# One-2-3-45/One-2-3-45

Hardware: NVIDIA H100
Metric: sec/mesh end-to-end (256x256 in) (lower is better)
Workload: dtype f16

## Files before the change

include/o2345.h:

```cpp
#ifndef O2345_H_
#define O2345_H_

#include <stddef.h>
#include <stdint.h>

#ifdef __cplusplus
extern "C" {
#endif

#define O2345_OK 0
#define O2345_EINVAL (-1)
#define O2345_ECUDA (-2)
#define O2345_EUNSUPPORTED (-3)

#define O2345_ABI_VERSION 5

typedef void* o2345_stream_t;

int o2345_abi_version(void);
int o2345_last_error(char* buf, size_t n);
int o2345_device_info(int* major, int* minor, int* sms);


#define O2345_SDF_PE 39
#define O2345_SDF_HID 128
#define O2345_SDF_LAT 16
#define O2345_SDF_IN1 144
#define O2345_SDF_PACK_FLOATS (39 * 128 + 128 + 2 * (144 * 128 + 128) + 128 * 144 + 128 * 48)

int o2345_sdf_pack_weights(const float* w0, const float* b0, const float* w1, const float* b1,
                           const float* w2, const float* b2, float* pack, o2345_stream_t stream);

#define O2345_PTS_EXPLICIT 0
#define O2345_PTS_LATTICE 1
#define O2345_PTS_RAYS 2

typedef struct o2345_points {
  int mode;
  const float* pts;
  const float* lin;
  int R;
  const float* rays_o;
  const float* rays_d;
  const float* z;
  int S;
  int z_stride;
} o2345_points;

#define O2345_SDF_FP32 0
#define O2345_SDF_TC_SPLIT 1
int o2345_sdf_query(const o2345_points* src, int64_t n, const float* vol_cl, int D, const float* wpack,
                    const uint8_t* active, float inactive_sdf, int negate, int precision, float* sdf, float* feat,
                    float* latent, float* grad, o2345_stream_t stream);


int o2345_frustum_mask(const float* proj, int V, const float* origin, float voxel_size, int D, int sizeH,
                       int sizeW, int min_views, uint32_t* mask_bits, uint8_t* keep, o2345_stream_t stream);

int64_t o2345_compact_scratch_ints(int64_t n);
int o2345_compact(const uint8_t* flags, int64_t n, int32_t* rows, int32_t* index, int32_t* count,
                  int32_t* scratch, o2345_stream_t stream);

int o2345_costvol_gather(const float* feats_nhwc, int V, int h, int w, int sizeH, int sizeW, const float* proj,
                         const float* origin, float voxel_size, int D, const int32_t* rows, const int32_t* count,
                         int64_t max_rows, const uint32_t* mask_bits, float* cost, o2345_stream_t stream);

int o2345_dense_scatter(const float* feat, const int32_t* rows, const int32_t* count, int64_t max_rows, int D,
                        float* vol_cl, float* vol_cf, float* occ, o2345_stream_t stream);

int o2345_occ_nearest(const o2345_points* src, int64_t n, const float* occ, int D, uint8_t* out,
                      o2345_stream_t stream);


int o2345_sdf_voxels(const float* occ, const float* vol_cl, int D, const float* origin, float voxel_size,
                     const float* wpack, int precision, float* sdf_vol, o2345_stream_t stream);

int o2345_prune_by_sdf(const float* sdf, const float* occ, int D, const float* ladder, int n_ladder, float* scratch,
                       float* minabs, int32_t* counts, o2345_stream_t stream);
int o2345_prune_select(const float* minabs, int64_t n, float threshold, uint8_t* keep, o2345_stream_t stream);
int o2345_clear_flags(const int32_t* rows, const int32_t* idx, int64_t n, uint8_t* flags, o2345_stream_t stream);
int o2345_gather_rows(const int32_t* rows, int64_t n, int D, const float* vol_cf, int C, float* coords, float* feats,
                      o2345_stream_t stream);

int o2345_lod_children(const float* pre_coords, int64_t n, int D1, const uint8_t* frustum_keep, uint8_t* keep,
                       int32_t* parent, int32_t* err_scratch, o2345_stream_t stream);

int o2345_costvol_gather_lod(const float* feats_nhwc, int C, int V, int h, int w, int sizeH, int sizeW, const float* proj,
                             const float* origin, float voxel_size, int D, const int32_t* rows, const int32_t* count,
                             int64_t max_rows, const uint32_t* mask_bits, const int32_t* parent, const float* pre_feats,
                             float* cost, o2345_stream_t stream);


int o2345_sp_coarsen(const int32_t* fine_index, int Ef, const int32_t* fine_rows, const int32_t* fine_count,
                     int64_t max_fine, int Ec, uint8_t* coarse_flags, int32_t* cmin_scratch,
                     o2345_stream_t stream);

int o2345_sp_conv(const float* in_feats, const int32_t* in_index, int Ein, const int32_t* out_rows,
                  const int32_t* out_count, int64_t max_out, int Eout, int mode, const float* kernel, int Cin,
                  int Cout, float* out_raw, double* stats, o2345_stream_t stream);

int o2345_sp_bn_relu(const float* x, const int32_t* count, int64_t max_rows, int C, const double* stats,
                     const float* gamma, const float* beta, float eps, const float* skip, float* out,
                     o2345_stream_t stream);

int o2345_mc_classify(const float* u, int R, float iso, uint8_t* cases, uint8_t* cell_flags, uint8_t* edge_flags,
                      o2345_stream_t stream);
int o2345_mc_vertices(const float* u, int R, float iso, const int32_t* edges, const int32_t* count,
                      int64_t max_verts, double* verts, o2345_stream_t stream);
int64_t o2345_scan_scratch_ints(int64_t n);
int o2345_mc_tri_offsets(const uint8_t* cases, const int32_t* cells, const int32_t* count, int64_t max_cells,
                         const uint8_t* n_tri_table, int32_t* offsets, int32_t* total, int32_t* scratch,
                         o2345_stream_t stream);
int o2345_mc_triangles(const uint8_t* cases, int R, const int32_t* cells, const int32_t* count, int64_t max_cells,
                       const int32_t* tri_offsets, const int8_t* tri_table, const uint8_t* n_tri_table,
                       const int8_t* edge_owner, const int32_t* vert_index, int32_t* tris, o2345_stream_t stream);

typedef struct o2345_view4 {
  float* ptr;
  int64_t sn, sc, sh, sw;
  int c0;
} o2345_view4;

int o2345_conv2d(const float* in, int N, int Cin, int H, int W, const float* weight, const float* bias, int Cout,
                 int K, int stride, int pad, float* out, double* stats, o2345_stream_t stream);
int o2345_abn_apply(const float* x, int N, int C, int H, int W, const double* stats, const float* gamma,
                    const float* beta, float eps, float slope, const o2345_view4* out, o2345_stream_t stream);
int o2345_upsample_bilinear(const float* x, int N, int C, int H, int W, int factor, const float* add,
                            const o2345_view4* out, o2345_stream_t stream);


int o2345_ray_upsample(const float* rays_o, const float* rays_d, int64_t R, const float* z, const float* sdf,
                       int S, float inv_s, const float* occ, int D, const float* u, int n_new, float* new_z,
                       o2345_stream_t stream);
int o2345_ray_merge(const float* z, const float* sdf, int S, const float* new_z, const float* new_sdf, int n_new,
                    int64_t R, float* out_z, float* out_sdf, o2345_stream_t stream);
int o2345_ray_midpoints(const float* rays_o, const float* rays_d, int64_t R, const float* z, int S,
                        float sample_dist, const float* occ, int D, float* mid_z, float* dists, uint8_t* active,
                        o2345_stream_t stream);

#define O2345_MAP_CH 60
#define O2345_RNET_PACK_FLOATS 19664

typedef struct o2345_views {
  int V, H, W;
  const float* maps;
  const float* proj;
  const float* centers;
  float sizeW, sizeH;
} o2345_views;

#define O2345_BLEND_FP32 0
#define O2345_BLEND_TC_FP16 1
int o2345_render_blend(const o2345_points* src, int64_t n, const uint8_t* active, const float* vol_cl,
                       const float* occ, int D, const o2345_views* views, int dir_mode, const float* query_center,
                       const float* dirs, const float* rnet_pack, int precision, float* rgb, int32_t* nvalid,
                       o2345_stream_t stream);

int o2345_ray_composite(const float* rays_d, int64_t R, int S, const float* mid_z, const float* dists,
                        const float* sdf, const float* grad, const float* color, const uint8_t* active,
                        const int32_t* nvalid, float inv_s, float alpha_inter_ratio, int has_background,
                        float background, float* color_out, float* depth_out, float* weights_out, float* cdf_out,
                        float* alpha_out, float* weights_sum_out, uint8_t* color_mask_out, o2345_stream_t stream);

typedef struct {
  const float* bias;
  const void* residual;
  const void* rowbias;
  int64_t rowbias_ld;
  int rows_per_group;
  int act;
  float alpha;
  int out_f32;
  float* colstats;
  int stats_rows_per_group;
} o2345_epilogue;

int o2345_gemm_f16(const void* A, const void* B, void* C, int M, int N, int K, int64_t lda, int64_t ldb,
                   int64_t ldc, int nh, int nb, int64_t stride_a_h, int64_t stride_a_b, int64_t stride_b_h,
                   int64_t stride_b_b, int64_t stride_c_h, int64_t stride_c_b, const o2345_epilogue* ep ,
                   float* splitk_ws, int64_t ws_floats, o2345_stream_t stream);

int o2345_last_trap(char* buf, size_t n);

void o2345_debug_gemm_force(int ctas, int bn, int splits);
void o2345_debug_gemm_persist(int mode, int min_tiles);
void o2345_debug_gemm_model(const float* seven);

void o2345_debug_gemm_trace(long long* device_buf16);

int o2345_conv3x3_f16(const void* x, int B, int H, int W, int C, const void* weight, int N, void* out, int64_t ldc,
                      const o2345_epilogue* ep, float* splitk_ws, int64_t ws_floats, o2345_stream_t stream);

int o2345_conv_up2x_f16(const void* x, int B, int H, int W, int C, const void* weight4, int N, void* out, int64_t ldc,
                        const o2345_epilogue* ep, float* splitk_ws, int64_t ws_floats, o2345_stream_t stream);

int64_t o2345_groupnorm_scratch_floats(int B, int G);
int o2345_groupnorm_stats(const void* x, int B, int HW, int C, int G, float eps, const float* gamma, const float* beta,
                          float* scratch, float* scale, float* shift, o2345_stream_t stream);
int o2345_groupnorm_apply(const void* x, int B, int HW, int C, int G, float eps, const float* gamma, const float* beta, int act,
                          void* out, o2345_stream_t stream);
void o2345_debug_groupnorm_cluster(int cl);
int o2345_norm_act_im2col(const void* x, int B, int H, int W, int C, int ksize, int stride, int upsample, int pad_lo,
                          const float* scale, const float* shift, int act, void* out, o2345_stream_t stream);
int o2345_norm_act_im2col_stats(const void* x, int B, int H, int W, int C, int ksize, int stride, int upsample, int pad_lo,
                                const float* stats_a, int Ca, const float* stats_b, int G, float eps, const float* gamma,
                                const float* beta, int act, void* out, o2345_stream_t stream);
int o2345_layernorm_rows(const void* x, int64_t M, int C, float eps, const float* gamma, const float* beta, void* y,
                         o2345_stream_t stream);
int o2345_softmax_rows(const void* s, int64_t rows, int n, void* p, o2345_stream_t stream);
int o2345_attention_f16(const void* q, const void* k, const void* v, int B, int N, int H, int d, int ld, void* out,
                        int ldo, float scale, o2345_stream_t stream);
int o2345_geglu(const void* x, int64_t M, int I, void* y, o2345_stream_t stream);
int o2345_silu(const void* x, int64_t n, void* y, o2345_stream_t stream);
int o2345_transpose_tokens(const void* x, int B, int N, int C, void* y, o2345_stream_t stream);
int o2345_timestep_embedding(const float* t, int B, int dim, void* out, o2345_stream_t stream);
int o2345_add_channel_bias(void* y, const void* e, int B, int HW, int C, int lde, o2345_stream_t stream);
int o2345_copy_channels(const void* src, int64_t M, int C, void* dst, int ldd, int off, o2345_stream_t stream);
int o2345_nchw_f32_to_cl_f16(const float* x, int B, int C, int HW, void* y, int ldy, int off, o2345_stream_t stream);
int o2345_cl_f16_to_nchw_f32(const void* x, int B, int C, int HW, int ldx, float* y, o2345_stream_t stream);
int o2345_cfg_ddim_update(const float* x, const float* eps, const float* noise, int64_t n, float scale, float a_t,
                          float a_prev, float sigma_t, float sqrt_one_minus_at, float* x_prev, float* pred_x0,
                          o2345_stream_t stream);

int o2345_clip_patches(const float* x, int B, int H, int W, int res, int patch, const float* mean3, const float* std3, int kp,
                       void* out, o2345_stream_t stream);
int o2345_clip_add_positions(void* tok, const float* cls, const float* pos, int B, int N, int d, o2345_stream_t stream);

#ifdef __cplusplus
}
#endif
#endif
```

one-2-3-45_b200/csrc/gemm_tc.cu:

```cuda
#include <cuda.h>
#include <stdlib.h>
#include <cuda_fp16.h>

#include "common.cuh"
#include "wgmma.cuh"

namespace o2345 {
namespace {

constexpr int BM = 128, BK = 64;
constexpr int EPI_WARPS = 8;
constexpr int EPI_THREADS = 32 * EPI_WARPS;
constexpr int GEMM_THREADS = 128 + EPI_THREADS;
constexpr uint64_t WAIT_LIMIT_NS = 4000000000ull;
constexpr int MAX_CLUSTER = 8;
constexpr int RES_PREFETCH = 8;

enum { WAIT_EMPTY = 1, WAIT_FULL = 2 };

struct TrapRecord {
  unsigned long long magic;
  int tag, stage, bx, by, bz, rank, M, N, K, bn, mode, splits, conv;
};
constexpr unsigned long long TRAP_MAGIC = 0x6f32333435545250ull;

__device__ __forceinline__ uint32_t smem_u32(const void* p) { return (uint32_t)__cvta_generic_to_shared(p); }

__device__ __forceinline__ void mbar_init(uint64_t* bar, uint32_t count) {
  asm volatile("mbarrier.init.shared::cta.b64 [%0], %1;" ::"r"(smem_u32(bar)), "r"(count));
}
__device__ __forceinline__ void mbar_expect_tx(uint64_t* bar, uint32_t bytes) {
  asm volatile("mbarrier.arrive.expect_tx.shared::cta.b64 _, [%0], %1;" ::"r"(smem_u32(bar)), "r"(bytes) : "memory");
}
__device__ __forceinline__ void mbar_arrive(uint64_t* bar) {
  asm volatile("mbarrier.arrive.shared::cta.b64 _, [%0];" ::"r"(smem_u32(bar)) : "memory");
}
__device__ __forceinline__ uint32_t mbar_try(uint64_t* bar, uint32_t parity) {
  uint32_t done;
  asm volatile(
      "{\n\t.reg .pred p;\n\t"
      "mbarrier.try_wait.parity.shared::cta.b64 p, [%1], %2;\n\t"
      "selp.u32 %0, 1, 0, p;\n\t}"
      : "=r"(done)
      : "r"(smem_u32(bar)), "r"(parity)
      : "memory");
  return done;
}
__device__ __forceinline__ uint64_t global_ns() {
  uint64_t t;
  asm volatile("mov.u64 %0, %%globaltimer;" : "=l"(t));
  return t;
}
__device__ __forceinline__ void tma_load_2d(void* dst, const CUtensorMap* map, uint64_t* bar, int c0, int c1) {
  asm volatile(
      "cp.async.bulk.tensor.2d.shared::cluster.global.mbarrier::complete_tx::bytes [%0], [%1, {%3, %4}], [%2];"
      ::"r"(smem_u32(dst)), "l"(map), "r"(smem_u32(bar)), "r"(c0), "r"(c1)
      : "memory");
}
__device__ __forceinline__ void tma_load_4d(void* dst, const CUtensorMap* map, uint64_t* bar, int c0, int c1, int c2, int c3) {
  asm volatile(
      "cp.async.bulk.tensor.4d.shared::cluster.global.mbarrier::complete_tx::bytes [%0], [%1, {%3, %4, %5, %6}], [%2];"
      ::"r"(smem_u32(dst)), "l"(map), "r"(smem_u32(bar)), "r"(c0), "r"(c1), "r"(c2), "r"(c3)
      : "memory");
}
__device__ __forceinline__ uint32_t cluster_ctarank() {
  uint32_t r;
  asm volatile("mov.u32 %0, %%cluster_ctarank;" : "=r"(r));
  return r;
}
__device__ __forceinline__ void cluster_sync_all() {
  asm volatile("barrier.cluster.arrive.release.aligned;\n\tbarrier.cluster.wait.acquire.aligned;" ::: "memory");
}
__device__ __forceinline__ void epi_bar() { asm volatile("bar.sync 1, 256;" ::: "memory"); }

__host__ __device__ constexpr int acc_ld(int bn) { return bn + 4; }
__device__ __forceinline__ void acc_ld32(const float* src, uint32_t (&r)[32]) {
#pragma unroll
  for (int i = 0; i < 8; ++i) {
    const float4 v = reinterpret_cast<const float4*>(src)[i];
    r[4 * i] = __float_as_uint(v.x), r[4 * i + 1] = __float_as_uint(v.y), r[4 * i + 2] = __float_as_uint(v.z), r[4 * i + 3] = __float_as_uint(v.w);
  }
}

struct GemmParams {
  int M, N, K;
  int64_t ldc;
  int nh;
  int64_t stride_c_h, stride_c_b;
  const float* bias;
  const __half* rowbias;
  int64_t rowbias_ld;
  int rows_per_group;
  const __half* residual;
  void* C;
  int out_f32;
  int act;
  float alpha;
  int batched;
  int conv, cC, cH, cW, cblocks;
  int ctaps, ctx, cox, coy, up, upa, upb;
  int splits;
  float* ws;
  int persist;
  float* colstats;
  int stats_rpg, stats_groups;
  long long* trace;
  TrapRecord* diag;
  int bn, mode;
};

__device__ __forceinline__ void stamp(const GemmParams& p, int slot) {
  if (p.trace && blockIdx.x == 0 && blockIdx.y == 0 && blockIdx.z == 0) p.trace[slot] = clock64();
}
__device__ __forceinline__ void stamp_ns(const GemmParams& p, int slot, bool any_z = false) {
  if (p.trace && blockIdx.x == 0 && blockIdx.y == 0 && (any_z || blockIdx.z == 0)) p.trace[slot] = (long long)global_ns();
}

__device__ __forceinline__ int64_t out_row(const GemmParams& p, int row) {
  if (!p.up) return row;
  const int x = row % p.cW, t = row / p.cW, y = t % p.cH, b = t / p.cH;
  return ((int64_t)b * (2 * p.cH) + 2 * y + p.upa) * (2 * p.cW) + 2 * x + p.upb;
}

__device__ __noinline__ void wait_timed_out(const GemmParams& p, int tag, int stage) {
  if (p.diag) {
    TrapRecord* d = p.diag;
    d->tag = tag, d->stage = stage, d->bx = blockIdx.x, d->by = blockIdx.y, d->bz = blockIdx.z, d->rank = (int)cluster_ctarank();
    d->M = p.M, d->N = p.N, d->K = p.K, d->bn = p.bn, d->mode = p.mode, d->splits = p.splits, d->conv = p.conv;
    __threadfence_system();
    d->magic = TRAP_MAGIC;
    __threadfence_system();
  }
  __trap();
}
__device__ __forceinline__ void mbar_wait(uint64_t* bar, uint32_t parity, const GemmParams& p, int tag, int stage) {
  if (mbar_try(bar, parity)) return;
  const uint64_t t0 = global_ns();
  uint32_t spins = 0;
  while (!mbar_try(bar, parity))
    if (((++spins) & 255u) == 0 && global_ns() - t0 > WAIT_LIMIT_NS) wait_timed_out(p, tag, stage);
}

__device__ __forceinline__ float gelu_erf(float x) { return 0.5f * x * (1.f + erff(x * 0.70710678118654752f)); }
__device__ __forceinline__ float gelu_erf_fast(float x) {
  const float z = fabsf(x) * 0.70710678118654752f;
  const float t = __fdividef(1.f, fmaf(0.3275911f, z, 1.f));
  const float poly = t * fmaf(t, fmaf(t, fmaf(t, fmaf(t, 1.061405429f, -1.453152027f), 1.421413741f), -0.284496736f), 0.254829592f);
  float e;
  asm("ex2.approx.ftz.f32 %0, %1;" : "=f"(e) : "f"(-z * z * 1.4426950408889634f));
  const float erf_abs = fmaf(-poly, e, 1.f);
  return 0.5f * x * (1.f + copysignf(erf_abs, x));
}
__device__ __forceinline__ float apply_act(float x, int act) {
  if (act == 1) return x / (1.f + __expf(-x));
  if (act == 2) return gelu_erf(x);
  if (act == 4) return x / (1.f + __expf(-1.702f * x));
  return x;
}

__device__ __forceinline__ void store8(const GemmParams& p, int64_t off, const float (&v)[8]) {
  if (p.out_f32) {
    float* o = reinterpret_cast<float*>(p.C) + off;
    *reinterpret_cast<float4*>(o) = make_float4(v[0], v[1], v[2], v[3]);
    *reinterpret_cast<float4*>(o + 4) = make_float4(v[4], v[5], v[6], v[7]);
  } else {
    __half2 h[4];
#pragma unroll
    for (int e = 0; e < 4; ++e) h[e] = __floats2half2_rn(v[2 * e], v[2 * e + 1]);
    *reinterpret_cast<uint4*>(reinterpret_cast<__half*>(p.C) + off) = *reinterpret_cast<uint4*>(h);
  }
}

__device__ __forceinline__ void epilogue_chunk(const GemmParams& p, const uint32_t (&r)[32], int row, int64_t crow, int col0) {
  const __half* rb = p.rowbias ? p.rowbias + (int64_t)(row / p.rows_per_group) * p.rowbias_ld : nullptr;
  if (p.act == 3) {
    if (col0 >= p.N) return;
    float v[16];
#pragma unroll
    for (int e = 0; e < 16; ++e) {
      float a = __uint_as_float(r[e]) * p.alpha, g = __uint_as_float(r[16 + e]) * p.alpha;
      if (p.bias) a += __ldg(p.bias + col0 + e), g += __ldg(p.bias + col0 + 16 + e);
      v[e] = a * gelu_erf(g);
    }
    const int64_t o = crow + (col0 >> 1);
    float lo[8], hi[8];
#pragma unroll
    for (int e = 0; e < 8; ++e) lo[e] = v[e], hi[e] = v[8 + e];
    store8(p, o, lo);
    store8(p, o + 8, hi);
    return;
  }
#pragma unroll
  for (int j = 0; j < 32; j += 8) {
    const int col = col0 + j;
    if (col >= p.N) break;
    float v[8];
    const bool full = col + 8 <= p.N;
    if (full && rb) {
      uint4 q = *reinterpret_cast<const uint4*>(rb + col);
      const __half* h = reinterpret_cast<const __half*>(&q);
#pragma unroll
      for (int e = 0; e < 8; ++e) v[e] = __half2float(h[e]);
    } else {
#pragma unroll
      for (int e = 0; e < 8; ++e) v[e] = (rb && col + e < p.N) ? __half2float(rb[col + e]) : 0.f;
    }
#pragma unroll
    for (int e = 0; e < 8; ++e) {
      float x = fmaf(__uint_as_float(r[j + e]), p.alpha, v[e]);
      if (p.bias && col + e < p.N) x += __ldg(p.bias + col + e);
      v[e] = apply_act(x, p.act);
    }
    if (full && (p.ldc & 7) == 0) {
      if (p.residual) {
        uint4 q = *reinterpret_cast<const uint4*>(p.residual + crow + col);
        const __half* h = reinterpret_cast<const __half*>(&q);
#pragma unroll
        for (int e = 0; e < 8; ++e) v[e] += __half2float(h[e]);
      }
      store8(p, crow + col, v);
    } else {
      for (int e = 0; e < 8 && col + e < p.N; ++e) {
        float x = v[e];
        if (p.residual) x += __half2float(p.residual[crow + col + e]);
        if (p.out_f32) reinterpret_cast<float*>(p.C)[crow + col + e] = x;
        else reinterpret_cast<__half*>(p.C)[crow + col + e] = __float2half_rn(x);
      }
    }
  }
}

__device__ __forceinline__ void splitk_partial(const GemmParams& p, const uint32_t (&r)[32], int split, int row, int col0) {
  float* w = p.ws + ((int64_t)split * p.M + row) * p.N + col0;
  if ((p.N & 3) == 0) {
#pragma unroll
    for (int e = 0; e < 32; e += 4)
      if (col0 + e < p.N)
        __stcg(reinterpret_cast<float4*>(w + e), make_float4(__uint_as_float(r[e]), __uint_as_float(r[e + 1]),
                                                              __uint_as_float(r[e + 2]), __uint_as_float(r[e + 3])));
  } else {
#pragma unroll
    for (int e = 0; e < 32; ++e)
      if (col0 + e < p.N) __stcg(w + e, __uint_as_float(r[e]));
  }
}

template <int BN>
__device__ __forceinline__ void splitk_finalize(const GemmParams& p, int m0, int n0, int z, int te, float* sstat) {
  const bool vec = (p.N % 8) == 0 && (p.ldc % 8) == 0 && (!p.rowbias || (p.rowbias_ld % 8) == 0);
  const int64_t plane = (int64_t)p.M * p.N;
  const bool stats = p.colstats != nullptr && vec && !p.out_f32;
  if (stats) {
    for (int i = te; i < 4 * BN; i += EPI_THREADS) sstat[i] = 0.f;
    epi_bar();
  }
  if (vec) {
    constexpr int PPR = BN / 8;
    constexpr int NP = BM * PPR;
    const int share = (NP + p.splits - 1) / p.splits;
    const int i1 = min(NP, (z + 1) * share);
    constexpr bool FIXED_COLS = (EPI_THREADS % PPR) == 0;
    float bcol[8];
#pragma unroll
    for (int e = 0; e < 8; ++e) bcol[e] = 0.f;
    if (FIXED_COLS && p.bias) {
      const int i0 = z * share + te, col = n0 + (i0 - (i0 / PPR) * PPR) * 8;
      if (col < p.N) {
        const float4 b0 = __ldg(reinterpret_cast<const float4*>(p.bias + col)), b1 = __ldg(reinterpret_cast<const float4*>(p.bias + col + 4));
        bcol[0] = b0.x, bcol[1] = b0.y, bcol[2] = b0.z, bcol[3] = b0.w, bcol[4] = b1.x, bcol[5] = b1.y, bcol[6] = b1.z, bcol[7] = b1.w;
      }
    }
    for (int i = z * share + te; i < i1; i += EPI_THREADS) {
      const int rl = i / PPR, row = m0 + rl, col = n0 + (i - rl * PPR) * 8;
      if (row >= p.M || col >= p.N) continue;
      const int64_t woff = (int64_t)row * p.N + col, o = out_row(p, row) * p.ldc + col;
      uint4 qb = make_uint4(0u, 0u, 0u, 0u), qr = make_uint4(0u, 0u, 0u, 0u);
      if (p.rowbias) qb = *reinterpret_cast<const uint4*>(p.rowbias + (int64_t)(row / p.rows_per_group) * p.rowbias_ld + col);
      if (p.residual) qr = *reinterpret_cast<const uint4*>(p.residual + o);
      if (!FIXED_COLS && p.bias) {
        const float4 b0 = __ldg(reinterpret_cast<const float4*>(p.bias + col)), b1 = __ldg(reinterpret_cast<const float4*>(p.bias + col + 4));
        bcol[0] = b0.x, bcol[1] = b0.y, bcol[2] = b0.z, bcol[3] = b0.w, bcol[4] = b1.x, bcol[5] = b1.y, bcol[6] = b1.z, bcol[7] = b1.w;
      }
      float v[8];
#pragma unroll
      for (int e = 0; e < 8; ++e) v[e] = 0.f;
      for (int s = 0; s < p.splits; s += 4) {
        float4 a[4], b[4];
#pragma unroll
        for (int t = 0; t < 4; ++t) {
          const bool on = s + t < p.splits;
          const float4* w = reinterpret_cast<const float4*>(p.ws + (int64_t)(s + t) * plane + woff);
          a[t] = on ? __ldcg(w) : make_float4(0.f, 0.f, 0.f, 0.f);
          b[t] = on ? __ldcg(w + 1) : make_float4(0.f, 0.f, 0.f, 0.f);
        }
#pragma unroll
        for (int t = 0; t < 4; ++t) {
          v[0] += a[t].x, v[1] += a[t].y, v[2] += a[t].z, v[3] += a[t].w;
          v[4] += b[t].x, v[5] += b[t].y, v[6] += b[t].z, v[7] += b[t].w;
        }
      }
      const __half* hb = reinterpret_cast<const __half*>(&qb);
#pragma unroll
      for (int e = 0; e < 8; ++e) {
        const float x = fmaf(v[e], p.alpha, p.rowbias ? __half2float(hb[e]) : 0.f) + bcol[e];
        v[e] = apply_act(x, p.act);
      }
      if (p.residual) {
        const __half* h = reinterpret_cast<const __half*>(&qr);
#pragma unroll
        for (int e = 0; e < 8; ++e) v[e] += __half2float(h[e]);
      }
      store8(p, o, v);
      if (stats) {
        float* acc = sstat + (row / p.stats_rpg - m0 / p.stats_rpg) * 2 * BN + (col - n0);
#pragma unroll
        for (int e = 0; e < 8; ++e) {
          const float x = __half2float(__float2half_rn(v[e]));
          atomicAdd(acc + e, x), atomicAdd(acc + BN + e, x * x);
        }
      }
    }
    if (stats) {
      epi_bar();
      const int g0 = m0 / p.stats_rpg;
      const int last_row = m0 + BM - 1 < p.M ? m0 + BM - 1 : p.M - 1;
      const int ng = last_row / p.stats_rpg - g0 + 1;
      for (int i = te; i < ng * 2 * BN; i += EPI_THREADS) {
        const int gi = i / (2 * BN), rem = i - gi * 2 * BN, mom = rem / BN, c = rem - mom * BN;
        if (n0 + c < p.N && sstat[i] != 0.f) atomicAdd(p.colstats + ((int64_t)(g0 + gi) * 2 + mom) * p.N + n0 + c, sstat[i]);
      }
    }
    return;
  }
  const int share = (BM * BN + p.splits - 1) / p.splits;
  const int i1 = min(BM * BN, (z + 1) * share);
  for (int i = z * share + te; i < i1; i += EPI_THREADS) {
    const int rl = i / BN, row = m0 + rl, col = n0 + (i - rl * BN);
    if (row >= p.M || col >= p.N) continue;
    float x = 0.f;
    for (int s = 0; s < p.splits; ++s) x += __ldcg(p.ws + (int64_t)s * plane + (int64_t)row * p.N + col);
    x *= p.alpha;
    if (p.rowbias) x += __half2float(p.rowbias[(int64_t)(row / p.rows_per_group) * p.rowbias_ld + col]);
    if (p.bias) x += __ldg(p.bias + col);
    x = apply_act(x, p.act);
    const int64_t o = out_row(p, row) * p.ldc + col;
    if (p.residual) x += __half2float(p.residual[o]);
    if (p.out_f32) reinterpret_cast<float*>(p.C)[o] = x;
    else reinterpret_cast<__half*>(p.C)[o] = __float2half_rn(x);
  }
}

constexpr int EPI_RB_GROUPS = 8;
__host__ __device__ constexpr int epi_smem_bytes(int bn) { return bn * 4 + EPI_RB_GROUPS * bn * 2; }
__host__ __device__ constexpr int col_split(int bn) { return ((bn / 2 + 31) / 32) * 32; }

template <int BN>
__device__ __forceinline__ void epilogue_preload(const GemmParams& p, int m0, int n0, float* sbias, __half* srb, int te) {
  for (int i = te; i < BN; i += EPI_THREADS) sbias[i] = (p.bias && n0 + i < p.N) ? __ldg(p.bias + n0 + i) : 0.f;
  if (p.rowbias) {
    const int g0 = m0 / p.rows_per_group;
    const int last = (m0 + BM - 1 < p.M ? m0 + BM - 1 : p.M - 1) / p.rows_per_group;
    const int ng = last - g0 + 1;
    if (ng >= 1 && ng <= EPI_RB_GROUPS)
      for (int i = te; i < ng * BN; i += EPI_THREADS) {
        const int gi = i / BN, c = i - gi * BN;
        srb[i] = (n0 + c < p.N) ? p.rowbias[(int64_t)(g0 + gi) * p.rowbias_ld + n0 + c] : __float2half(0.f);
      }
  }
  epi_bar();
}

template <int ACT>
__device__ __forceinline__ float act_fn(float x) {
  if (ACT == 1) return __fdividef(x, 1.f + __expf(-x));
  if (ACT == 2) return gelu_erf(x);
  if (ACT == 4) return __fdividef(x, 1.f + __expf(-1.702f * x));
  return x;
}

template <int ACT>
__device__ __forceinline__ void stage_rows(const GemmParams& p, const float* acc_row, uint8_t* mine, int n0, int c_lo, int c_hi,
                                           const float* sbias, const __half* rb, bool rb_smem) {
#pragma unroll 1
  for (int c0 = c_lo; c0 < c_hi; c0 += 32) {
    if (n0 + c0 >= p.N) break;
    uint32_t r[32];
    acc_ld32(acc_row + c0, r);
    if (ACT == 3) {
      __half2 h[8];
#pragma unroll
      for (int e = 0; e < 16; e += 2) {
        float a0 = fmaf(__uint_as_float(r[e]), p.alpha, sbias[c0 + e]), a1 = fmaf(__uint_as_float(r[e + 1]), p.alpha, sbias[c0 + e + 1]);
        float g0 = fmaf(__uint_as_float(r[16 + e]), p.alpha, sbias[c0 + 16 + e]);
        float g1 = fmaf(__uint_as_float(r[17 + e]), p.alpha, sbias[c0 + 17 + e]);
        h[e >> 1] = __floats2half2_rn(a0 * gelu_erf_fast(g0), a1 * gelu_erf_fast(g1));
      }
      uint4* d = reinterpret_cast<uint4*>(mine + (c0 - c_lo));
      d[0] = reinterpret_cast<uint4*>(h)[0], d[1] = reinterpret_cast<uint4*>(h)[1];
    } else {
#pragma unroll
      for (int j = 0; j < 32; j += 8) {
        float v[8];
        const float4 b0 = *reinterpret_cast<const float4*>(sbias + c0 + j), b1 = *reinterpret_cast<const float4*>(sbias + c0 + j + 4);
        v[0] = b0.x, v[1] = b0.y, v[2] = b0.z, v[3] = b0.w, v[4] = b1.x, v[5] = b1.y, v[6] = b1.z, v[7] = b1.w;
        if (rb && (rb_smem || n0 + c0 + j + 8 <= p.N)) {
          uint4 q = *reinterpret_cast<const uint4*>(rb + c0 + j);
          const __half* hq = reinterpret_cast<const __half*>(&q);
#pragma unroll
          for (int e = 0; e < 8; ++e) v[e] += __half2float(hq[e]);
        }
        __half2 h[4];
#pragma unroll
        for (int e = 0; e < 8; e += 2) {
          float x0 = fmaf(__uint_as_float(r[j + e]), p.alpha, v[e]), x1 = fmaf(__uint_as_float(r[j + e + 1]), p.alpha, v[e + 1]);
          h[e >> 1] = __floats2half2_rn(act_fn<ACT>(x0), act_fn<ACT>(x1));
        }
        *reinterpret_cast<uint4*>(mine + (c0 - c_lo + j) * 2) = *reinterpret_cast<uint4*>(h);
      }
    }
  }
}

struct WarpOut {
  int outc, stride, ppr, total, ocol0, nout;
};
template <int MODE>
__device__ __forceinline__ WarpOut warp_out(const GemmParams& p, int n0, int c_lo, int c_hi) {
  constexpr bool geglu = MODE == 1;
  WarpOut g;
  g.outc = geglu ? (c_hi - c_lo) >> 1 : (c_hi - c_lo);
  g.stride = g.outc * 2 + 16;
  g.ppr = g.outc >> 3;
  g.total = 32 * g.ppr;
  g.ocol0 = geglu ? (n0 + c_lo) >> 1 : n0 + c_lo;
  g.nout = geglu ? p.N >> 1 : p.N;
  return g;
}

__device__ __forceinline__ void prefetch_residual(const GemmParams& p, const WarpOut& g, int lane, int row0,
                                                  uint4 (&resq)[RES_PREFETCH]) {
#pragma unroll
  for (int u = 0; u < RES_PREFETCH; ++u) {
    resq[u] = make_uint4(0u, 0u, 0u, 0u);
    const int pp = lane + 32 * u;
    if (p.residual && pp < g.total) {
      const int rl = pp / g.ppr, ci = pp - rl * g.ppr;
      const int grow = row0 + rl, col = g.ocol0 + ci * 8;
      if (grow < p.M && col < g.nout) resq[u] = *reinterpret_cast<const uint4*>(p.residual + out_row(p, grow) * p.ldc + col);
    }
  }
}

__device__ __forceinline__ uint4 add_h8(uint4 v, uint4 q) {
  __half2* a = reinterpret_cast<__half2*>(&v);
  const __half2* b = reinterpret_cast<const __half2*>(&q);
#pragma unroll
  for (int e = 0; e < 4; ++e) {
    float2 fa = __half22float2(a[e]), fb = __half22float2(b[e]);
    a[e] = __floats2half2_rn(fa.x + fb.x, fa.y + fb.y);
  }
  return v;
}

template <int BN, int MODE>
__device__ __forceinline__ void epilogue_staged(const GemmParams& p, const WarpOut& g, const float* acc_row, uint8_t* slab, int lane,
                                                int m0, int row0, int n0, int c_lo, int c_hi, const float* sbias, const __half* srb,
                                                const uint4 (&resq)[RES_PREFETCH]) {
  const int row = row0 + lane;
  const __half* rb = nullptr;
  bool rb_smem = false;
  if (MODE != 1 && p.rowbias) {
    const int rr = row < p.M ? row : p.M - 1;
    const int g0 = m0 / p.rows_per_group, last = (m0 + BM - 1 < p.M ? m0 + BM - 1 : p.M - 1) / p.rows_per_group;
    rb_smem = last - g0 + 1 <= EPI_RB_GROUPS;
    rb = rb_smem ? srb + (rr / p.rows_per_group - g0) * BN : p.rowbias + (int64_t)(rr / p.rows_per_group) * p.rowbias_ld + n0;
  }
  uint8_t* mine = slab + lane * g.stride;
  if (MODE == 0) {
    stage_rows<0>(p, acc_row, mine, n0, c_lo, c_hi, sbias, rb, rb_smem);
  } else if (MODE == 1) {
    stage_rows<3>(p, acc_row, mine, n0, c_lo, c_hi, sbias, rb, rb_smem);
  } else {
    switch (p.act) {
      case 1: stage_rows<1>(p, acc_row, mine, n0, c_lo, c_hi, sbias, rb, rb_smem); break;
      case 2: stage_rows<2>(p, acc_row, mine, n0, c_lo, c_hi, sbias, rb, rb_smem); break;
      default: stage_rows<4>(p, acc_row, mine, n0, c_lo, c_hi, sbias, rb, rb_smem); break;
    }
  }
  __syncwarp();
  __half* C = reinterpret_cast<__half*>(p.C);
#pragma unroll
  for (int u = 0; u < RES_PREFETCH; ++u) {
    const int pp = lane + 32 * u;
    if (pp < g.total) {
      const int rl = pp / g.ppr, ci = pp - rl * g.ppr;
      const int grow = row0 + rl, col = g.ocol0 + ci * 8;
      if (grow < p.M && col < g.nout) {
        uint4 v = *reinterpret_cast<const uint4*>(slab + rl * g.stride + ci * 16);
        if (p.residual) {
          v = add_h8(v, resq[u]);
          if (p.colstats) *reinterpret_cast<uint4*>(slab + rl * g.stride + ci * 16) = v;
        }
        *reinterpret_cast<uint4*>(C + out_row(p, grow) * p.ldc + col) = v;
      }
    }
  }
  constexpr int UN = 4;
  for (int base = lane + 32 * RES_PREFETCH; base < g.total; base += 32 * UN) {
    uint4 v[UN], q[UN];
    int64_t o[UN];
    bool ok[UN];
#pragma unroll
    for (int u = 0; u < UN; ++u) {
      const int pp = base + 32 * u;
      const int rl = pp / g.ppr, ci = pp - rl * g.ppr;
      const int grow = row0 + rl, col = g.ocol0 + ci * 8;
      ok[u] = pp < g.total && grow < p.M && col < g.nout;
      o[u] = out_row(p, grow) * p.ldc + col;
      if (ok[u]) {
        v[u] = *reinterpret_cast<const uint4*>(slab + rl * g.stride + ci * 16);
        if (p.residual) q[u] = *reinterpret_cast<const uint4*>(p.residual + o[u]);
      }
    }
#pragma unroll
    for (int u = 0; u < UN; ++u) {
      if (!ok[u]) continue;
      if (p.residual) {
        v[u] = add_h8(v[u], q[u]);
        if (p.colstats) {
          const int pp = base + 32 * u;
          const int rl = pp / g.ppr, ci = pp - rl * g.ppr;
          *reinterpret_cast<uint4*>(slab + rl * g.stride + ci * 16) = v[u];
        }
      }
      *reinterpret_cast<uint4*>(C + o[u]) = v[u];
    }
  }
  if (MODE == 0 && p.colstats) {
    __syncwarp();
    const int nrows = p.M - row0 < 32 ? p.M - row0 : 32;
    if (nrows > 0) {
      float* ssum = p.colstats + (int64_t)(row0 / p.stats_rpg) * 2 * g.nout;
      for (int cp = lane; 2 * cp < g.outc; cp += 32) {
        const int col = g.ocol0 + 2 * cp;
        if (col >= g.nout) break;
        float s0 = 0.f, s1 = 0.f, q0 = 0.f, q1 = 0.f;
        if (nrows == 32) {
#pragma unroll 8
          for (int r = 0; r < 32; ++r) {
            const float2 f = __half22float2(*reinterpret_cast<const __half2*>(slab + r * g.stride + cp * 4));
            s0 += f.x, s1 += f.y, q0 = fmaf(f.x, f.x, q0), q1 = fmaf(f.y, f.y, q1);
          }
        } else {
          for (int r = 0; r < nrows; ++r) {
            const float2 f = __half22float2(*reinterpret_cast<const __half2*>(slab + r * g.stride + cp * 4));
            s0 += f.x, s1 += f.y, q0 = fmaf(f.x, f.x, q0), q1 = fmaf(f.y, f.y, q1);
          }
        }
        atomicAdd(ssum + col, s0), atomicAdd(ssum + col + 1, s1);
        atomicAdd(ssum + g.nout + col, q0), atomicAdd(ssum + g.nout + col + 1, q1);
      }
    }
  }
}

__host__ __device__ constexpr int epi_slab_bytes(int bn) { return EPI_WARPS * 32 * (col_split(bn) * 2 + 16); }
constexpr int smem_bytes(int bn, int stages) {
  return stages * (BM * BK * 2 + bn * BK * 2) + epi_slab_bytes(bn) + 2 * stages * 8 + 16 + epi_smem_bytes(bn) + 1024;
}

template <int BN>
__device__ __forceinline__ void produce_stage(const GemmParams& p, const CUtensorMap* tmA, const CUtensorMap* tmB, uint8_t* a_dst,
                                              uint8_t* b_dst, uint64_t* full_bar, int kb, int m0, int n0, int bz) {
  mbar_expect_tx(full_bar, BM * BK * 2 + BN * BK * 2);
  if (p.conv) {
    const int tap = kb / p.cblocks, c0 = (kb - tap * p.cblocks) * BK;
    const int x0 = m0 % p.cW, y0 = (m0 / p.cW) % p.cH, b0 = m0 / (p.cW * p.cH);
    tma_load_4d(a_dst, tmA, full_bar, c0, x0 + tap % p.ctx + p.cox, y0 + tap / p.ctx + p.coy, b0);
    tma_load_2d(b_dst, tmB, full_bar, tap * p.cC + c0, n0);
  } else if (p.batched) {
    tma_load_4d(a_dst, tmA, full_bar, kb * BK, m0, bz % p.nh, bz / p.nh);
    tma_load_4d(b_dst, tmB, full_bar, kb * BK, n0, bz % p.nh, bz / p.nh);
  } else {
    tma_load_2d(a_dst, tmA, full_bar, kb * BK, m0);
    tma_load_2d(b_dst, tmB, full_bar, kb * BK, n0);
  }
}

template <int BN>
__device__ __forceinline__ void acc_store(float* acc, const float (&d)[BN / 2], int row0, int t) {
  const int r = row0 + 16 * (t >> 5) + ((t & 31) >> 2), c = 2 * (t & 3);
#pragma unroll
  for (int j = 0; j < BN / 8; ++j) {
    *reinterpret_cast<float2*>(acc + r * acc_ld(BN) + 8 * j + c) = make_float2(d[4 * j], d[4 * j + 1]);
    *reinterpret_cast<float2*>(acc + (r + 8) * acc_ld(BN) + 8 * j + c) = make_float2(d[4 * j + 2], d[4 * j + 3]);
  }
}

template <int BN, int STAGES, int MODE>
__global__ void __launch_bounds__(GEMM_THREADS, 1)
gemm_tc_kernel(const __grid_constant__ CUtensorMap tmA, const __grid_constant__ CUtensorMap tmB, const __grid_constant__ GemmParams p) {
  extern __shared__ __align__(1024) uint8_t smem_raw[];
  uint8_t* smem = reinterpret_cast<uint8_t*>((reinterpret_cast<uintptr_t>(smem_raw) + 1023) & ~(uintptr_t)1023);
  constexpr int A_BYTES = BM * BK * 2, B_BYTES = BN * BK * 2;
  static_assert(B_BYTES % 1024 == 0, "stage bases must stay 1024-byte aligned for SWIZZLE_128B");
  static_assert(BN % 32 == 0 && BN >= 64 && BN <= 256, "tile width: a multiple of 32 (GEGLU chunks, 32-column epilogue reads)");
  static_assert(BM * acc_ld(BN) * 4 <= STAGES * (A_BYTES + B_BYTES), "the accumulator tile must fit in the operand ring");
  constexpr int CSPLIT = col_split(BN);
  uint8_t* sA = smem;
  uint8_t* sB = smem + STAGES * A_BYTES;
  uint8_t* slabs = sB + STAGES * B_BYTES;
  uint64_t* full = reinterpret_cast<uint64_t*>(slabs + epi_slab_bytes(BN));
  uint64_t* empty = full + STAGES;
  float* sbias = reinterpret_cast<float*>((reinterpret_cast<uintptr_t>(empty + STAGES) + 15) & ~(uintptr_t)15);
  __half* srb = reinterpret_cast<__half*>(sbias + BN);
  float* acc = reinterpret_cast<float*>(smem);

  const int warp = threadIdx.x >> 5, lane = threadIdx.x & 31;
  if (threadIdx.x == 0) stamp(p, 0), stamp_ns(p, 16);
  const int bz = blockIdx.z;
  const int nk = p.conv ? p.ctaps * p.cblocks : (p.K + BK - 1) / BK;
  const bool split = MODE == 3 && p.splits > 1;
  int kb0 = 0, kb1 = nk;
  if (split) {
    kb0 = (int)((int64_t)nk * bz / p.splits);
    kb1 = (int)((int64_t)nk * (bz + 1) / p.splits);
  }

  if (threadIdx.x == 0) {
    asm volatile("prefetch.tensormap [%0];" ::"l"(&tmA) : "memory");
    asm volatile("prefetch.tensormap [%0];" ::"l"(&tmB) : "memory");
    for (int s = 0; s < STAGES; ++s) mbar_init(full + s, 1), mbar_init(empty + s, 2);
    asm volatile("fence.mbarrier_init.release.cluster;" ::: "memory");
    asm volatile("fence.proxy.async.shared::cta;" ::: "memory");
  }
  __syncthreads();
  pdl_wait();
  pdl_trigger();
  if (threadIdx.x == 0) stamp(p, 1);

  const int tiles_m = (p.M + BM - 1) / BM, tiles = tiles_m * ((p.N + BN - 1) / BN);
  const bool persist = MODE != 3 && p.persist;
  uint32_t cnt = 0;
  for (int t = persist ? blockIdx.x : blockIdx.y * tiles_m + blockIdx.x; t < tiles; t += persist ? gridDim.x : tiles) {
  const int m0 = (t % tiles_m) * BM, n0 = (t / tiles_m) * BN;
  if (warp < 4) {
    if (threadIdx.x == 0) {
      asm volatile("fence.proxy.async.shared::cta;" ::: "memory");
      for (int kb = kb0; kb < kb1; ++kb) {
        const uint32_t c = cnt + (kb - kb0);
        const int s = c % STAGES;
        const uint32_t ph = (c / STAGES) & 1;
        mbar_wait(empty + s, ph ^ 1, p, WAIT_EMPTY, s);
        produce_stage<BN>(p, &tmA, &tmB, sA + s * A_BYTES, sB + s * B_BYTES, full + s, kb, m0, n0, bz);
        if (kb == kb0) stamp(p, 2);
      }
      stamp(p, 3);
    }
    __syncwarp();
  } else {
    const int wg = (warp >> 2) - 1, e = warp - 4, quarter = e & 3, te = threadIdx.x - 128;
    const int c_lo = e < 4 ? 0 : CSPLIT, c_hi = e < 4 ? CSPLIT : BN;
    const int row0 = m0 + quarter * 32;
    if (MODE != 3) epilogue_preload<BN>(p, m0, n0, sbias, srb, te);
    {
      float d[BN / 2];
#pragma unroll
      for (int i = 0; i < BN / 2; ++i) d[i] = 0.f;
      for (int kb = kb0; kb < kb1; ++kb) {
        const uint32_t c = cnt + (kb - kb0);
        const int s = c % STAGES;
        const uint32_t ph = (c / STAGES) & 1;
        mbar_wait(full + s, ph, p, WAIT_FULL, s);
        if (kb == kb0 && te == 0) stamp(p, 4);
        const uint32_t a0 = smem_u32(sA + s * A_BYTES) + wg * (64 * 128), b0 = smem_u32(sB + s * B_BYTES);
        wg::fence();
#pragma unroll
        for (int k = 0; k < BK / 16; ++k)
          wg::mma_f16<BN>(d, wg::desc_sw128(a0 + k * 32), wg::desc_sw128(b0 + k * 32), 1);
        wg::commit();
        wg::wait<1>();
        if (kb > kb0 && (threadIdx.x & 127) == 0) mbar_arrive(empty + (c - 1) % STAGES);
      }
      wg::wait<0>();
      if ((threadIdx.x & 127) == 0) mbar_arrive(empty + (cnt + kb1 - kb0 - 1) % STAGES);
      if (te == 0) stamp(p, 5);
      epi_bar();
      acc_store<BN>(acc, d, 64 * wg, threadIdx.x & 127);
    }
    epi_bar();
    if (te == 0) stamp(p, 6);
    const float* acc_row = acc + (quarter * 32 + lane) * acc_ld(BN);
    if (MODE != 3) {
      const WarpOut g = warp_out<MODE>(p, n0, c_lo, c_hi);
      uint4 resq[RES_PREFETCH];
      prefetch_residual(p, g, lane, row0, resq);
      epilogue_staged<BN, MODE>(p, g, acc_row, slabs + e * 32 * (CSPLIT * 2 + 16), lane, m0, row0, n0, c_lo, c_hi, sbias, srb, resq);
    } else {
      const int row = row0 + lane;
      if (split) {
        if (te == 0) stamp_ns(p, 17);
#pragma unroll 1
        for (int c0 = c_lo; c0 < c_hi; c0 += 32) {
          uint32_t r[32];
          acc_ld32(acc_row + c0, r);
          if (row < p.M) splitk_partial(p, r, bz, row, n0 + c0);
        }
        if (te == 0) stamp_ns(p, 18);
      } else {
        const int64_t crow = (p.batched ? (int64_t)(bz % p.nh) * p.stride_c_h + (int64_t)(bz / p.nh) * p.stride_c_b : 0) +
                             out_row(p, row < p.M ? row : 0) * p.ldc;
#pragma unroll 1
        for (int c0 = c_lo; c0 < c_hi; c0 += 32) {
          uint32_t r[32];
          acc_ld32(acc_row + c0, r);
          if (row < p.M) epilogue_chunk(p, r, row, crow, n0 + c0);
        }
      }
    }
    if (te == 0) stamp(p, 7);
  }
  cnt += kb1 - kb0;
  __syncthreads();
  }
  if (split) {
    cluster_sync_all();
    if (warp >= 4) {
      if (threadIdx.x == 128) stamp_ns(p, 21, true);
      splitk_finalize<BN>(p, blockIdx.x * BM, blockIdx.y * BN, bz, threadIdx.x - 128, reinterpret_cast<float*>(smem));
      if (threadIdx.x == 128) stamp_ns(p, 22, true);
    }
  }
  if (threadIdx.x == 0) stamp(p, 8);
}

typedef CUresult (*EncodeTiledFn)(CUtensorMap*, CUtensorMapDataType, cuuint32_t, void*, const cuuint64_t*, const cuuint64_t*,
                                  const cuuint32_t*, const cuuint32_t*, CUtensorMapInterleave, CUtensorMapSwizzle,
                                  CUtensorMapL2promotion, CUtensorMapFloatOOBfill);

EncodeTiledFn encode_fn() {
  static EncodeTiledFn fn = nullptr;
  if (!fn) {
    void* p = nullptr;
    cudaDriverEntryPointQueryResult q;
    if (cudaGetDriverEntryPoint("cuTensorMapEncodeTiled", &p, cudaEnableDefault, &q) == cudaSuccess && q == cudaDriverEntryPointSuccess)
      fn = reinterpret_cast<EncodeTiledFn>(p);
  }
  return fn;
}

int make_map(CUtensorMap* m, const void* ptr, int64_t rows, int64_t K, int64_t ld, int nh, int nb, int64_t sh, int64_t sb,
             int box_rows) {
  EncodeTiledFn fn = encode_fn();
  if (!fn) { set_error("cuTensorMapEncodeTiled entry point not available"); return O2345_ECUDA; }
  cuuint64_t dims[4] = {(cuuint64_t)K, (cuuint64_t)rows, (cuuint64_t)(nh > 0 ? nh : 1), (cuuint64_t)(nb > 0 ? nb : 1)};
  cuuint64_t strides[3] = {(cuuint64_t)ld * 2, (cuuint64_t)sh * 2, (cuuint64_t)sb * 2};
  cuuint32_t box[4] = {(cuuint32_t)BK, (cuuint32_t)box_rows, 1, 1};
  cuuint32_t estr[4] = {1, 1, 1, 1};
  int rank = nh > 0 ? 4 : 2;
  CUresult r = fn(m, CU_TENSOR_MAP_DATA_TYPE_FLOAT16, rank, const_cast<void*>(ptr), dims, strides, box, estr,
                  CU_TENSOR_MAP_INTERLEAVE_NONE, CU_TENSOR_MAP_SWIZZLE_128B, CU_TENSOR_MAP_L2_PROMOTION_L2_256B,
                  CU_TENSOR_MAP_FLOAT_OOB_FILL_NONE);
  if (r != CUDA_SUCCESS) { set_error("cuTensorMapEncodeTiled failed with %d (rows=%lld K=%lld ld=%lld)", (int)r, (long long)rows, (long long)K, (long long)ld); return O2345_ECUDA; }
  return O2345_OK;
}

TrapRecord* g_diag = nullptr;
bool g_diag_tried = false;
TrapRecord* diag_buffer(cudaStream_t st) {
  if (!g_diag_tried) {
    cudaStreamCaptureStatus cs = cudaStreamCaptureStatusNone;
    if (cudaStreamIsCapturing(st, &cs) != cudaSuccess || cs != cudaStreamCaptureStatusNone) {
      cudaGetLastError();
      return g_diag;
    }
    g_diag_tried = true;
    void* h = nullptr;
    if (cudaHostAlloc(&h, sizeof(TrapRecord), cudaHostAllocMapped | cudaHostAllocPortable) == cudaSuccess) {
      memset(h, 0, sizeof(TrapRecord));
      g_diag = reinterpret_cast<TrapRecord*>(h);
    } else {
      cudaGetLastError();
    }
  }
  return g_diag;
}

struct Config {
  int bn, splits;
  int persist;
};

int g_force[3] = {-1, 0, 0};
int g_persist = 0;
int g_persist_min_tiles = 0;
void read_force_env() {
  if (g_force[0] >= 0) return;
  g_force[0] = g_force[1] = g_force[2] = 0;
  const char* e = getenv("O2345_GEMM_FORCE");
  if (e) sscanf(e, "%d,%d,%d", &g_force[0], &g_force[1], &g_force[2]);
}

float g_model[7] = {40.f, 0.5f, 6300.f, 5.f, 3.f, 4.f, 1.f};
float predict_us(int M, int N, int nk, int bn, int splits) {
  const float bw_sm = g_model[0], alpha = g_model[1], cap = g_model[2], fixed = g_model[3], epi = g_model[4], so0 = g_model[5],
              so1 = g_model[6], cyc_per_us = 1750.f;
  const int tiles = cdiv(M, BM) * cdiv(N, bn);
  const int n = tiles * splits;
  const int kb = cdiv(nk, splits);
  const float bytes_cta = (float)kb * (float)(BM * BK * 2 + bn * BK * 2);
  const int sms = sm_count();
  const int rounds = cdiv(n, sms);
  float f = (float)(n - sms) / (float)sms;
  f = f < 0.f ? 0.f : (f > 1.f ? 1.f : f);
  const float t_sm = (float)rounds * bytes_cta / (bw_sm * (1.f + alpha * f));
  const float t_fabric = (float)n * bytes_cta / cap;
  const float t_mma = (float)rounds * (float)kb * 4.f * (float)bn;
  float t = t_sm > t_fabric ? t_sm : t_fabric;
  if (t_mma > t) t = t_mma;
  float us = fixed + t / cyc_per_us + epi * (float)bn / 160.f * (float)cdiv(n, sms);
  if (splits > 1) us += so0 + so1 * (float)splits * (float)bn / 128.f;
  return us;
}

Config pick_config(const GemmParams& p, int nk, bool can_split, int64_t ws_floats) {
  read_force_env();
  Config c;
  const int M = p.M, N = p.N;
  c.persist = 0;
  if (p.batched) {
    c.bn = N <= 64 ? 64 : 128, c.splits = 1;
    return c;
  }
  static const int kBn[4] = {64, 128, 160, 256};
  static const int kSplits[6] = {1, 2, 3, 4, 6, 8};
  const bool split_ok = can_split && p.act != 3 && p.ws && 2 * (int64_t)M * N <= ws_floats;
  const int max_planes = split_ok ? (int)(ws_floats / ((int64_t)M * N)) : 1;
  float best = 1e30f;
  c.bn = 128, c.splits = 1;
  for (int bi = 0; bi < 4; ++bi) {
    const int bn = kBn[bi];
    if (bn > 64 && N <= 64) continue;
    if (g_force[1] > 0 && bn != g_force[1]) continue;
    for (int si = 0; si < 6; ++si) {
      const int sp = kSplits[si];
      if (g_force[2] > 0 && sp != (g_force[2] > nk ? nk : g_force[2])) continue;
      if (sp > 1 && (!split_ok || sp > max_planes || sp > MAX_CLUSTER || nk / sp < 3)) continue;
      const float us = predict_us(M, N, nk, bn, sp);
      if (us < best) best = us, c.bn = bn, c.splits = sp;
    }
  }
  if (best > 1e29f) {
    c.bn = (g_force[1] == 64 || g_force[1] == 128 || g_force[1] == 160 || g_force[1] == 256) ? g_force[1] : 128;
    c.splits = 1;
  }
  const int tiles = cdiv(M, BM) * cdiv(N, c.bn);
  const int min_tiles = g_persist_min_tiles > 0 ? g_persist_min_tiles : 4 * sm_count();
  c.persist = c.splits == 1 && (g_persist == 1 || (g_persist == 0 && tiles >= min_tiles));
  return c;
}

int pick_mode(const GemmParams& p, const Config& c) {
  const int nout = p.act == 3 ? p.N / 2 : p.N;
  const bool staged = !p.out_f32 && c.splits <= 1 && !p.batched && (nout % 8) == 0 && (p.ldc % 8) == 0 && ((uintptr_t)p.C % 16) == 0 &&
                      (!p.residual || ((uintptr_t)p.residual % 16) == 0);
  if (!staged) return 3;
  return p.act == 0 ? 0 : (p.act == 3 ? 1 : 2);
}

long long* g_trace = nullptr;

template <int BN, int STAGES, int MODE>
int launch(const CUtensorMap& a, const CUtensorMap& b, GemmParams p, int batch, int persist, cudaStream_t st) {
  constexpr int SMEM = smem_bytes(BN, STAGES);
  static_assert(SMEM <= 227 * 1024, "one CTA per SM");
  static PerDeviceOnce attr;
  if (attr.need())
    O2345_CUDA(cudaFuncSetAttribute(gemm_tc_kernel<BN, STAGES, MODE>, cudaFuncAttributeMaxDynamicSharedMemorySize, SMEM));
  p.bn = BN, p.mode = MODE;
  p.diag = diag_buffer(st);
  const int splits = (MODE == 3 && batch == 0 && p.splits > 1) ? p.splits : 1;
  p.splits = splits;
  dim3 grid(cdiv(p.M, BM), cdiv(p.N, BN), batch > 0 ? batch : splits);
  p.persist = MODE != 3 && batch == 0 && splits == 1 && persist;
  if (p.persist) {
    const int tiles = (int)grid.x * (int)grid.y;
    grid = dim3(tiles < sm_count() ? tiles : sm_count(), 1, 1);
  }
  O2345_CUDA(launch_pdl_cluster(gemm_tc_kernel<BN, STAGES, MODE>, grid, dim3(GEMM_THREADS), (size_t)SMEM, st, 1, splits, a, b, p));
  O2345_LAUNCH_CHECK();
  return O2345_OK;
}

template <int BN, int STAGES>
int launch_mode(int mode, const CUtensorMap& a, const CUtensorMap& b, const GemmParams& p, int batch, int persist, cudaStream_t st) {
  switch (mode) {
    case 0: return launch<BN, STAGES, 0>(a, b, p, batch, persist, st);
    case 1: return launch<BN, STAGES, 1>(a, b, p, batch, persist, st);
    case 2: return launch<BN, STAGES, 2>(a, b, p, batch, persist, st);
    default: return launch<BN, STAGES, 3>(a, b, p, batch, persist, st);
  }
}

int dispatch(const Config& c, int mode, const CUtensorMap& a, const CUtensorMap& b, const GemmParams& p, int batch, cudaStream_t st) {
  if (p.colstats && mode == 3 && c.splits <= 1) {
    set_error("o2345_gemm_f16: column statistics need the staged fp16 epilogue (16-byte aligned C / residual) or split-K");
    return O2345_EUNSUPPORTED;
  }
  if (c.bn == 64) return launch_mode<64, 6>(mode, a, b, p, batch, c.persist, st);
  if (c.bn == 128) return launch_mode<128, 5>(mode, a, b, p, batch, c.persist, st);
  if (c.bn == 160) return launch_mode<160, 4>(mode, a, b, p, batch, c.persist, st);
  return launch_mode<256, 3>(mode, a, b, p, batch, c.persist, st);
}

int fill_epilogue(GemmParams& p, const o2345_epilogue* ep, int M, int N, int64_t ldc) {
  p.bias = nullptr, p.rowbias = nullptr, p.rowbias_ld = 0, p.rows_per_group = 1, p.residual = nullptr;
  p.out_f32 = 0, p.act = 0, p.alpha = 1.f, p.trace = g_trace;
  p.colstats = nullptr, p.stats_rpg = 1, p.stats_groups = 0;
  p.diag = nullptr, p.bn = p.mode = 0;
  if (!ep) return O2345_OK;
  O2345_CHECK_ARG(ep->act >= 0 && ep->act <= 4, "unknown activation");
  O2345_CHECK_ARG(!ep->rowbias || (ep->rows_per_group > 0 && (ep->rowbias_ld % 8) == 0 && ((uintptr_t)ep->rowbias % 16) == 0),
                  "row bias: rows_per_group > 0, 16-byte aligned, row stride a multiple of 8");
  O2345_CHECK_ARG(ep->act != 3 || ((N % 32) == 0 && (ldc % 8) == 0 && !ep->residual && !ep->rowbias),
                  "GEGLU epilogue: N must be a multiple of 32, ldc of 8, no residual / row bias");
  p.bias = ep->bias, p.rowbias = reinterpret_cast<const __half*>(ep->rowbias), p.rowbias_ld = ep->rowbias_ld;
  p.rows_per_group = ep->rowbias ? ep->rows_per_group : 1;
  p.residual = reinterpret_cast<const __half*>(ep->residual), p.out_f32 = ep->out_f32, p.act = ep->act, p.alpha = ep->alpha;
  if (ep->colstats) {
    O2345_CHECK_ARG(ep->act == 0 && !ep->out_f32 && (N % 8) == 0 && (ldc % 8) == 0,
                    "column statistics: fp16 output without activation, N and ldc multiples of 8");
    O2345_CHECK_ARG(ep->stats_rows_per_group > 0 && ((ep->stats_rows_per_group % 128) == 0 || ep->stats_rows_per_group == 64),
                    "column statistics: rows per group must be 64 or a multiple of 128");
    p.colstats = ep->colstats, p.stats_rpg = ep->stats_rows_per_group, p.stats_groups = cdiv(M, ep->stats_rows_per_group);
  }
  return O2345_OK;
}

void set_workspace(GemmParams& p, float* ws, int64_t ws_floats) { p.ws = ws_floats > 0 ? ws : nullptr; }

}
}

using namespace o2345;

extern "C" void o2345_debug_gemm_trace(long long* device_buf16) { g_trace = device_buf16; }

extern "C" void o2345_debug_gemm_force(int ctas, int bn, int splits) {
  read_force_env();
  g_force[0] = ctas, g_force[1] = bn, g_force[2] = splits;
}


extern "C" void o2345_debug_gemm_persist(int mode, int min_tiles) { g_persist = mode, g_persist_min_tiles = min_tiles; }

extern "C" void o2345_debug_gemm_model(const float* seven) {
  for (int i = 0; i < 7; ++i) g_model[i] = seven[i];
}

extern "C" int o2345_last_trap(char* buf, size_t n) {
  if (!buf || n == 0) return O2345_EINVAL;
  buf[0] = 0;
  const TrapRecord* d = g_diag;
  if (!d || d->magic != TRAP_MAGIC) return 0;
  static const char* names[] = {"?", "empty (producer waiting for the MMA to free a stage)", "full (MMA issuer waiting for TMA bytes)",
                                };
  snprintf(buf, n,
           "gemm_tc_kernel<BN=%d, MODE=%d> M=%d N=%d K=%d conv=%d splits=%d: CTA (%d,%d,%d) rank %d gave up after 4 s "
           "on barrier '%s' stage %d",
           d->bn, d->mode, d->M, d->N, d->K, d->conv, d->splits, d->bx, d->by, d->bz, d->rank,
           names[d->tag >= 1 && d->tag <= 2 ? d->tag : 0], d->stage);
  return 1;
}

namespace o2345 {
namespace {
int conv_launch(const void* x, int B, int H, int W, int C, const void* weight, int N, void* out, int64_t ldc, const o2345_epilogue* ep,
                float* splitk_ws, int64_t ws_floats, int taps, int tx, int ox, int oy, int up, int upa, int upb, cudaStream_t st) {
  EncodeTiledFn fn = encode_fn();
  if (!fn) { set_error("cuTensorMapEncodeTiled entry point not available"); return O2345_ECUDA; }
  const int tw = W >= 128 ? 128 : W;
  const int th = W >= 128 ? 1 : (128 / W < H ? 128 / W : H);
  const int tb = 128 / (tw * th);
  CUtensorMap ma, mb;
  {
    cuuint64_t dims[4] = {(cuuint64_t)C, (cuuint64_t)W, (cuuint64_t)H, (cuuint64_t)B};
    cuuint64_t strides[3] = {(cuuint64_t)C * 2, (cuuint64_t)W * C * 2, (cuuint64_t)H * W * C * 2};
    cuuint32_t box[4] = {(cuuint32_t)BK, (cuuint32_t)tw, (cuuint32_t)th, (cuuint32_t)tb};
    cuuint32_t estr[4] = {1, 1, 1, 1};
    CUresult r = fn(&ma, CU_TENSOR_MAP_DATA_TYPE_FLOAT16, 4, const_cast<void*>(x), dims, strides, box, estr,
                    CU_TENSOR_MAP_INTERLEAVE_NONE, CU_TENSOR_MAP_SWIZZLE_128B, CU_TENSOR_MAP_L2_PROMOTION_L2_256B,
                    CU_TENSOR_MAP_FLOAT_OOB_FILL_NONE);
    if (r != CUDA_SUCCESS) { set_error("cuTensorMapEncodeTiled (conv activation) failed with %d", (int)r); return O2345_ECUDA; }
  }
  GemmParams p;
  p.M = B * H * W, p.N = N, p.K = taps * C, p.ldc = ldc, p.nh = 1, p.stride_c_h = 0, p.stride_c_b = 0, p.C = out;
  int rc = fill_epilogue(p, ep, p.M, N, ldc);
  if (rc) return rc;
  p.batched = 0, p.conv = 1, p.cC = C, p.cH = H, p.cW = W, p.cblocks = (C + BK - 1) / BK;
  p.ctaps = taps, p.ctx = tx, p.cox = ox, p.coy = oy, p.up = up, p.upa = upa, p.upb = upb;
  set_workspace(p, splitk_ws, ws_floats);
  const Config c = pick_config(p, taps * p.cblocks, true, ws_floats);
  p.splits = c.splits;
  rc = make_map(&mb, weight, N, taps * (int64_t)C, taps * (int64_t)C, 0, 0, 0, 0, c.bn);
  if (rc) return rc;
  return dispatch(c, pick_mode(p, c), ma, mb, p, 0, st);
}

bool conv_tiles(int H, int W) {
  return (W % 128) == 0 || ((128 % W) == 0 && (((int64_t)H * W >= 128 && (H % (128 / W)) == 0) || ((int64_t)H * W < 128 && (128 % (H * W)) == 0)));
}
}
}

extern "C" int o2345_conv3x3_f16(const void* x, int B, int H, int W, int C, const void* weight, int N, void* out, int64_t ldc,
                                 const o2345_epilogue* ep, float* splitk_ws, int64_t ws_floats, o2345_stream_t stream) {
  O2345_CHECK_ARG(x && weight && out, "null pointer");
  O2345_CHECK_ARG(B > 0 && H > 0 && W > 0 && C > 0 && (C % 8) == 0 && N > 0, "bad sizes (C must be a multiple of 8)");
  O2345_CHECK_ARG(conv_tiles(H, W),
                  "implicit 3x3 conv: the image must tile into 128-pixel boxes (W % 128 == 0, or 128 % W == 0 with "
                  "H % (128 / W) == 0, or 128 % (H * W) == 0)");
  O2345_CHECK_ARG(((uintptr_t)x % 16) == 0 && ((uintptr_t)weight % 16) == 0, "operands must be 16-byte aligned");
  return conv_launch(x, B, H, W, C, weight, N, out, ldc, ep, splitk_ws, ws_floats, 9, 3, -1, -1, 0, 0, 0, (cudaStream_t)stream);
}

extern "C" int o2345_conv_up2x_f16(const void* x, int B, int H, int W, int C, const void* weight4, int N, void* out, int64_t ldc,
                                   const o2345_epilogue* ep, float* splitk_ws, int64_t ws_floats, o2345_stream_t stream) {
  O2345_CHECK_ARG(x && weight4 && out, "null pointer");
  O2345_CHECK_ARG(B > 0 && H > 0 && W > 0 && C > 0 && (C % 8) == 0 && N > 0, "bad sizes (C must be a multiple of 8)");
  O2345_CHECK_ARG(conv_tiles(H, W), "up-sampling conv: the LOW-resolution image must tile into 128-pixel boxes (see o2345_conv3x3_f16)");
  O2345_CHECK_ARG(((uintptr_t)x % 16) == 0 && ((uintptr_t)weight4 % 16) == 0, "operands must be 16-byte aligned");
  O2345_CHECK_ARG(!ep || (!ep->residual && !ep->colstats && !ep->rowbias && ep->act != 3),
                  "up-sampling conv: bias / activation epilogues only (no residual, row bias, statistics, GEGLU)");
  O2345_CHECK_ARG((int64_t)B * 4 * H * W < (1ll << 31), "output rows must fit 31 bits");
  const __half* w = reinterpret_cast<const __half*>(weight4);
  for (int ph = 0; ph < 4; ++ph) {
    const int a = ph >> 1, b = ph & 1;
    int rc = conv_launch(x, B, H, W, C, w + (int64_t)ph * N * 4 * C, N, out, ldc, ep, splitk_ws, ws_floats, 4, 2, b - 1, a - 1, 1, a, b,
                         (cudaStream_t)stream);
    if (rc) return rc;
  }
  return O2345_OK;
}

extern "C" int o2345_gemm_f16(const void* A, const void* B, void* C, int M, int N, int K, int64_t lda, int64_t ldb,
                              int64_t ldc, int nh, int nb, int64_t stride_a_h, int64_t stride_a_b, int64_t stride_b_h,
                              int64_t stride_b_b, int64_t stride_c_h, int64_t stride_c_b, const o2345_epilogue* ep,
                              float* splitk_ws, int64_t ws_floats, o2345_stream_t stream) {
  O2345_CHECK_ARG(A && B && C, "null pointer");
  O2345_CHECK_ARG(M > 0 && N > 0 && K > 0 && nh >= 0 && (nh == 0 || nb >= 1), "bad sizes");
  O2345_CHECK_ARG((lda % 8) == 0 && (ldb % 8) == 0, "row strides of A and B must be multiples of 8 fp16 (16 bytes) for TMA");
  O2345_CHECK_ARG(((uintptr_t)A % 16) == 0 && ((uintptr_t)B % 16) == 0, "A and B must be 16-byte aligned");
  O2345_CHECK_ARG(nh == 0 || ((stride_a_h % 8) == 0 && (stride_a_b % 8) == 0 && (stride_b_h % 8) == 0 && (stride_b_b % 8) == 0),
                  "batch strides must be multiples of 8 fp16");
  GemmParams p;
  p.M = M, p.N = N, p.K = K, p.ldc = ldc, p.nh = nh > 0 ? nh : 1, p.stride_c_h = stride_c_h, p.stride_c_b = stride_c_b, p.C = C;
  int rc = fill_epilogue(p, ep, M, N, ldc);
  if (rc) return rc;
  O2345_CHECK_ARG(nh == 0 || (!p.rowbias && p.act != 3), "row bias / GEGLU are not available in batched mode");
  p.batched = nh > 0 ? 1 : 0;
  p.conv = 0, p.cC = p.cH = p.cW = p.cblocks = 0;
  p.ctaps = p.ctx = p.cox = p.coy = p.up = p.upa = p.upb = 0;
  set_workspace(p, splitk_ws, ws_floats);
  cudaStream_t st = (cudaStream_t)stream;
  const Config c = pick_config(p, cdiv(K, BK), nh == 0, ws_floats);
  p.splits = c.splits;
  CUtensorMap ma, mb;
  rc = make_map(&ma, A, M, K, lda, nh, nb, stride_a_h, stride_a_b, BM);
  if (rc) return rc;
  rc = make_map(&mb, B, N, K, ldb, nh, nb, stride_b_h, stride_b_b, c.bn);
  if (rc) return rc;
  return dispatch(c, pick_mode(p, c), ma, mb, p, nh > 0 ? nh * nb : 0, st);
}
```

one-2-3-45_b200/o2345/_lib.py:

```python
from __future__ import annotations

import ctypes as C
import functools
import os

HERE = os.path.dirname(os.path.abspath(__file__))
LIB_PATH = os.environ.get("O2345_LIB") or os.path.join(os.path.dirname(HERE), "lib", "libo2345_sm90.so")

c_fp = C.c_void_p
c_i64 = C.c_int64


class Points(C.Structure):
    _fields_ = [("mode", C.c_int), ("pts", c_fp), ("lin", c_fp), ("R", C.c_int), ("rays_o", c_fp),
                ("rays_d", c_fp), ("z", c_fp), ("S", C.c_int), ("z_stride", C.c_int)]


class View4(C.Structure):
    _fields_ = [("ptr", c_fp), ("sn", c_i64), ("sc", c_i64), ("sh", c_i64), ("sw", c_i64), ("c0", C.c_int)]


class Views(C.Structure):
    _fields_ = [("V", C.c_int), ("H", C.c_int), ("W", C.c_int), ("maps", c_fp), ("proj", c_fp),
                ("centers", c_fp), ("sizeW", C.c_float), ("sizeH", C.c_float)]


class Epilogue(C.Structure):
    _fields_ = [("bias", c_fp), ("residual", c_fp), ("rowbias", c_fp), ("rowbias_ld", c_i64), ("rows_per_group", C.c_int),
                ("act", C.c_int), ("alpha", C.c_float), ("out_f32", C.c_int), ("colstats", c_fp), ("stats_rows_per_group", C.c_int)]


PTS_EXPLICIT, PTS_LATTICE, PTS_RAYS = 0, 1, 2
BLEND_FP32, BLEND_TC_FP16 = 0, 1
SDF_FP32, SDF_TC_SPLIT = 0, 1
SDF_PACK_FLOATS = 39 * 128 + 128 + 2 * (144 * 128 + 128) + 128 * 144 + 128 * 48
RNET_PACK_FLOATS = 19664
MAP_CH = 60

_SIGS = {
    "o2345_abi_version": (C.c_int, []),
    "o2345_last_error": (C.c_int, [C.c_char_p, C.c_size_t]),
    "o2345_device_info": (C.c_int, [C.POINTER(C.c_int)] * 3),
    "o2345_sdf_pack_weights": (C.c_int, [c_fp] * 7 + [c_fp]),
    "o2345_sdf_query": (C.c_int, [C.POINTER(Points), c_i64, c_fp, C.c_int, c_fp, c_fp, C.c_float, C.c_int, C.c_int,
                                  c_fp, c_fp, c_fp, c_fp, c_fp]),
    "o2345_frustum_mask": (C.c_int, [c_fp, C.c_int, c_fp, C.c_float, C.c_int, C.c_int, C.c_int, C.c_int, c_fp,
                                     c_fp, c_fp]),
    "o2345_compact_scratch_ints": (c_i64, [c_i64]),
    "o2345_compact": (C.c_int, [c_fp, c_i64, c_fp, c_fp, c_fp, c_fp, c_fp]),
    "o2345_costvol_gather": (C.c_int, [c_fp, C.c_int, C.c_int, C.c_int, C.c_int, C.c_int, c_fp, c_fp, C.c_float,
                                       C.c_int, c_fp, c_fp, c_i64, c_fp, c_fp, c_fp]),
    "o2345_dense_scatter": (C.c_int, [c_fp, c_fp, c_fp, c_i64, C.c_int, c_fp, c_fp, c_fp, c_fp]),
    "o2345_sdf_voxels": (C.c_int, [c_fp, c_fp, C.c_int, c_fp, C.c_float, c_fp, C.c_int, c_fp, c_fp]),
    "o2345_prune_by_sdf": (C.c_int, [c_fp, c_fp, C.c_int, C.POINTER(C.c_float), C.c_int, c_fp, c_fp, c_fp, c_fp]),
    "o2345_prune_select": (C.c_int, [c_fp, c_i64, C.c_float, c_fp, c_fp]),
    "o2345_clear_flags": (C.c_int, [c_fp, c_fp, c_i64, c_fp, c_fp]),
    "o2345_gather_rows": (C.c_int, [c_fp, c_i64, C.c_int, c_fp, C.c_int, c_fp, c_fp, c_fp]),
    "o2345_lod_children": (C.c_int, [c_fp, c_i64, C.c_int, c_fp, c_fp, c_fp, c_fp, c_fp]),
    "o2345_costvol_gather_lod": (C.c_int, [c_fp, C.c_int, C.c_int, C.c_int, C.c_int, C.c_int, C.c_int, c_fp, c_fp, C.c_float,
                                           C.c_int, c_fp, c_fp, c_i64, c_fp, c_fp, c_fp, c_fp, c_fp]),
    "o2345_occ_nearest": (C.c_int, [C.POINTER(Points), c_i64, c_fp, C.c_int, c_fp, c_fp]),
    "o2345_sp_coarsen": (C.c_int, [c_fp, C.c_int, c_fp, c_fp, c_i64, C.c_int, c_fp, c_fp, c_fp]),
    "o2345_sp_conv": (C.c_int, [c_fp, c_fp, C.c_int, c_fp, c_fp, c_i64, C.c_int, C.c_int, c_fp, C.c_int, C.c_int,
                                c_fp, c_fp, c_fp]),
    "o2345_sp_bn_relu": (C.c_int, [c_fp, c_fp, c_i64, C.c_int, c_fp, c_fp, c_fp, C.c_float, c_fp, c_fp, c_fp]),
    "o2345_mc_classify": (C.c_int, [c_fp, C.c_int, C.c_float, c_fp, c_fp, c_fp, c_fp]),
    "o2345_mc_vertices": (C.c_int, [c_fp, C.c_int, C.c_float, c_fp, c_fp, c_i64, c_fp, c_fp]),
    "o2345_scan_scratch_ints": (c_i64, [c_i64]),
    "o2345_mc_tri_offsets": (C.c_int, [c_fp, c_fp, c_fp, c_i64, c_fp, c_fp, c_fp, c_fp, c_fp]),
    "o2345_mc_triangles": (C.c_int, [c_fp, C.c_int, c_fp, c_fp, c_i64, c_fp, c_fp, c_fp, c_fp, c_fp, c_fp, c_fp]),
    "o2345_conv2d": (C.c_int, [c_fp, C.c_int, C.c_int, C.c_int, C.c_int, c_fp, c_fp, C.c_int, C.c_int, C.c_int,
                               C.c_int, c_fp, c_fp, c_fp]),
    "o2345_abn_apply": (C.c_int, [c_fp, C.c_int, C.c_int, C.c_int, C.c_int, c_fp, c_fp, c_fp, C.c_float, C.c_float,
                                  C.POINTER(View4), c_fp]),
    "o2345_upsample_bilinear": (C.c_int, [c_fp, C.c_int, C.c_int, C.c_int, C.c_int, C.c_int, c_fp,
                                          C.POINTER(View4), c_fp]),
    "o2345_ray_upsample": (C.c_int, [c_fp, c_fp, c_i64, c_fp, c_fp, C.c_int, C.c_float, c_fp, C.c_int, c_fp,
                                     C.c_int, c_fp, c_fp]),
    "o2345_ray_merge": (C.c_int, [c_fp, c_fp, C.c_int, c_fp, c_fp, C.c_int, c_i64, c_fp, c_fp, c_fp]),
    "o2345_ray_midpoints": (C.c_int, [c_fp, c_fp, c_i64, c_fp, C.c_int, C.c_float, c_fp, C.c_int, c_fp, c_fp,
                                      c_fp, c_fp]),
    "o2345_render_blend": (C.c_int, [C.POINTER(Points), c_i64, c_fp, c_fp, c_fp, C.c_int, C.POINTER(Views),
                                     C.c_int, c_fp, c_fp, c_fp, C.c_int, c_fp, c_fp, c_fp]),
    "o2345_gemm_f16": (C.c_int, [c_fp, c_fp, c_fp, C.c_int, C.c_int, C.c_int, c_i64, c_i64, c_i64, C.c_int, C.c_int,
                                 c_i64, c_i64, c_i64, c_i64, c_i64, c_i64, C.POINTER(Epilogue), c_fp, c_i64, c_fp]),
    "o2345_debug_gemm_trace": (None, [c_fp]),
    "o2345_debug_gemm_force": (None, [C.c_int, C.c_int, C.c_int]),
    "o2345_debug_gemm_persist": (None, [C.c_int, C.c_int]),
    "o2345_debug_groupnorm_cluster": (None, [C.c_int]),
    "o2345_debug_gemm_model": (None, [C.POINTER(C.c_float)]),
    "o2345_last_trap": (C.c_int, [C.c_char_p, C.c_size_t]),
    "o2345_conv3x3_f16": (C.c_int, [c_fp, C.c_int, C.c_int, C.c_int, C.c_int, c_fp, C.c_int, c_fp, c_i64,
                                    C.POINTER(Epilogue), c_fp, c_i64, c_fp]),
    "o2345_conv_up2x_f16": (C.c_int, [c_fp, C.c_int, C.c_int, C.c_int, C.c_int, c_fp, C.c_int, c_fp, c_i64,
                                      C.POINTER(Epilogue), c_fp, c_i64, c_fp]),
    "o2345_groupnorm_scratch_floats": (c_i64, [C.c_int, C.c_int]),
    "o2345_groupnorm_stats": (C.c_int, [c_fp, C.c_int, C.c_int, C.c_int, C.c_int, C.c_float, c_fp, c_fp, c_fp, c_fp, c_fp,
                                        c_fp]),
    "o2345_groupnorm_apply": (C.c_int, [c_fp, C.c_int, C.c_int, C.c_int, C.c_int, C.c_float, c_fp, c_fp, C.c_int, c_fp, c_fp]),
    "o2345_norm_act_im2col": (C.c_int, [c_fp, C.c_int, C.c_int, C.c_int, C.c_int, C.c_int, C.c_int, C.c_int, C.c_int, c_fp, c_fp,
                                        C.c_int, c_fp, c_fp]),
    "o2345_norm_act_im2col_stats": (C.c_int, [c_fp, C.c_int, C.c_int, C.c_int, C.c_int, C.c_int, C.c_int, C.c_int, C.c_int, c_fp, C.c_int,
                                              c_fp, C.c_int, C.c_float, c_fp, c_fp, C.c_int, c_fp, c_fp]),
    "o2345_layernorm_rows": (C.c_int, [c_fp, c_i64, C.c_int, C.c_float, c_fp, c_fp, c_fp, c_fp]),
    "o2345_softmax_rows": (C.c_int, [c_fp, c_i64, C.c_int, c_fp, c_fp]),
    "o2345_attention_f16": (C.c_int, [c_fp, c_fp, c_fp, C.c_int, C.c_int, C.c_int, C.c_int, C.c_int, c_fp, C.c_int,
                                      C.c_float, c_fp]),
    "o2345_geglu": (C.c_int, [c_fp, c_i64, C.c_int, c_fp, c_fp]),
    "o2345_silu": (C.c_int, [c_fp, c_i64, c_fp, c_fp]),
    "o2345_transpose_tokens": (C.c_int, [c_fp, C.c_int, C.c_int, C.c_int, c_fp, c_fp]),
    "o2345_timestep_embedding": (C.c_int, [c_fp, C.c_int, C.c_int, c_fp, c_fp]),
    "o2345_add_channel_bias": (C.c_int, [c_fp, c_fp, C.c_int, C.c_int, C.c_int, C.c_int, c_fp]),
    "o2345_copy_channels": (C.c_int, [c_fp, c_i64, C.c_int, c_fp, C.c_int, C.c_int, c_fp]),
    "o2345_nchw_f32_to_cl_f16": (C.c_int, [c_fp, C.c_int, C.c_int, C.c_int, c_fp, C.c_int, C.c_int, c_fp]),
    "o2345_cl_f16_to_nchw_f32": (C.c_int, [c_fp, C.c_int, C.c_int, C.c_int, C.c_int, c_fp, c_fp]),
    "o2345_cfg_ddim_update": (C.c_int, [c_fp, c_fp, c_fp, c_i64, C.c_float, C.c_float, C.c_float, C.c_float, C.c_float,
                                        c_fp, c_fp, c_fp]),
    "o2345_clip_patches": (C.c_int, [c_fp, C.c_int, C.c_int, C.c_int, C.c_int, C.c_int, C.POINTER(C.c_float), C.POINTER(C.c_float),
                                     C.c_int, c_fp, c_fp]),
    "o2345_clip_add_positions": (C.c_int, [c_fp, c_fp, c_fp, C.c_int, C.c_int, C.c_int, c_fp]),
    "o2345_ray_composite": (C.c_int, [c_fp, c_i64, C.c_int, c_fp, c_fp, c_fp, c_fp, c_fp, c_fp, c_fp, C.c_float,
                                      C.c_float, C.c_int, C.c_float, c_fp, c_fp, c_fp, c_fp, c_fp, c_fp, c_fp, c_fp]),
}

EXPORTED = tuple(_SIGS)
ABI_VERSION = 5
_lib = None


class O2345Error(RuntimeError):
    pass


def load():
    global _lib
    if _lib is None:
        if not os.path.exists(LIB_PATH):
            raise O2345Error(f"{LIB_PATH} is missing: run `python one-2-3-45_b200/build.py` "
                             "(there is no CPU or PyTorch fallback for this path)")
        lib = C.CDLL(LIB_PATH)
        for name, (res, args) in _SIGS.items():
            fn = getattr(lib, name)
            fn.restype, fn.argtypes = res, args
        if lib.o2345_abi_version() != ABI_VERSION:
            raise O2345Error(f"{LIB_PATH} has ABI version {lib.o2345_abi_version()}, this binding expects {ABI_VERSION}: "
                             "rebuild with `python one-2-3-45_b200/build.py`")
        _lib = lib
    return _lib


def last_trap() -> str:
    buf = C.create_string_buffer(512)
    return buf.value.decode(errors="replace") if load().o2345_last_trap(buf, 512) == 1 else ""


def last_error() -> str:
    buf = C.create_string_buffer(512)
    load().o2345_last_error(buf, 512)
    return buf.value.decode(errors="replace")


_KERNELS_PER_CALL = {"o2345_compact": 3, "o2345_prune_by_sdf": 3, "o2345_sp_coarsen": 3, "o2345_mc_tri_offsets": 4, "o2345_conv_up2x_f16": 4}
_launches = 0


def reset_launches():
    global _launches
    _launches = 0


def add_launches(n: int):
    global _launches
    _launches += n


def launches() -> int:
    return _launches


def call(name, *args):
    global _launches
    rc = getattr(load(), name)(*args)
    if rc != 0:
        raise O2345Error(f"{name} failed with {rc}: {last_error()}")
    _launches += _KERNELS_PER_CALL.get(name, 1)
    return rc


def inference_only(fn):
    import torch

    @functools.wraps(fn)
    def wrap(self, *args, **kwargs):
        if torch.is_grad_enabled() and any(p.requires_grad for p in self.parameters()):
            raise RuntimeError(f"o2345 {type(self).__name__}.{fn.__name__} is inference-only: call it under torch.no_grad() or "
                               "freeze the parameters (requires_grad_(False)); training stays with the reference")
        with torch.no_grad():
            return fn(self, *args, **kwargs)
    return wrap
```

Measured before the change: 3.360.

## Add CTA-pair B-tile multicast and stage epilogue directly from MMA fragments

Adds an optional two-CTA cluster mode in which each CTA loads half of the B tile and multicasts it to its peer, halving B traffic from global memory. The epilogue now writes results straight from the wgmma register fragments into the output slabs, dropping the fp32 accumulator round trip through shared memory. Pipeline depth is now derived from the shared memory budget, which likely allows more stages. The pairing path adds cluster launch constraints, remote barrier arrivals and an occupancy query, and is gated behind a debug toggle.

After: 3.308, median of 6. 1.6% less time.

```diff
diff --git a/include/o2345.h b/include/o2345.h
--- a/include/o2345.h
+++ b/include/o2345.h
@@ -184,6 +184,7 @@
 
 void o2345_debug_gemm_force(int ctas, int bn, int splits);
 void o2345_debug_gemm_persist(int mode, int min_tiles);
+void o2345_debug_gemm_pair(int mode);
 void o2345_debug_gemm_model(const float* seven);
 
 void o2345_debug_gemm_trace(long long* device_buf16);
diff --git a/one-2-3-45_b200/csrc/gemm_tc.cu b/one-2-3-45_b200/csrc/gemm_tc.cu
--- a/one-2-3-45_b200/csrc/gemm_tc.cu
+++ b/one-2-3-45_b200/csrc/gemm_tc.cu
@@ -20,7 +20,7 @@
 
 struct TrapRecord {
   unsigned long long magic;
-  int tag, stage, bx, by, bz, rank, M, N, K, bn, mode, splits, conv;
+  int tag, stage, bx, by, bz, rank, peer, M, N, K, bn, mode, splits, conv;
 };
 constexpr unsigned long long TRAP_MAGIC = 0x6f32333435545250ull;
 
@@ -63,6 +63,20 @@
       ::"r"(smem_u32(dst)), "l"(map), "r"(smem_u32(bar)), "r"(c0), "r"(c1), "r"(c2), "r"(c3)
       : "memory");
 }
+__device__ __forceinline__ void tma_load_2d_mc(void* dst, const CUtensorMap* map, uint64_t* bar, int c0, int c1, uint16_t cta_mask) {
+  asm volatile(
+      "cp.async.bulk.tensor.2d.shared::cluster.global.mbarrier::complete_tx::bytes.multicast::cluster [%0], [%1, {%4, %5}], [%2], %3;"
+      ::"r"(smem_u32(dst)), "l"(map), "r"(smem_u32(bar)), "h"(cta_mask), "r"(c0), "r"(c1)
+      : "memory");
+}
+__device__ __forceinline__ void mbar_arrive_remote(uint64_t* bar, uint32_t rank) {
+  asm volatile(
+      "{\n\t.reg .b32 ra;\n\t"
+      "mapa.shared::cluster.u32 ra, %0, %1;\n\t"
+      "mbarrier.arrive.release.cluster.shared::cluster.b64 _, [ra];\n\t}"
+      ::"r"(smem_u32(bar)), "r"(rank)
+      : "memory");
+}
 __device__ __forceinline__ uint32_t cluster_ctarank() {
   uint32_t r;
   asm volatile("mov.u32 %0, %%cluster_ctarank;" : "=r"(r));
@@ -73,14 +87,8 @@
 }
 __device__ __forceinline__ void epi_bar() { asm volatile("bar.sync 1, 256;" ::: "memory"); }
 
-__host__ __device__ constexpr int acc_ld(int bn) { return bn + 4; }
-__device__ __forceinline__ void acc_ld32(const float* src, uint32_t (&r)[32]) {
-#pragma unroll
-  for (int i = 0; i < 8; ++i) {
-    const float4 v = reinterpret_cast<const float4*>(src)[i];
-    r[4 * i] = __float_as_uint(v.x), r[4 * i + 1] = __float_as_uint(v.y), r[4 * i + 2] = __float_as_uint(v.z), r[4 * i + 3] = __float_as_uint(v.w);
-  }
-}
+__device__ __forceinline__ int frag_row(int t) { return 16 * (t >> 5) + ((t & 31) >> 2); }
+__device__ __forceinline__ int frag_col(int t) { return 2 * (t & 3); }
 
 struct GemmParams {
   int M, N, K;
@@ -102,6 +110,7 @@
   int splits;
   float* ws;
   int persist;
+  int pair;
   float* colstats;
   int stats_rpg, stats_groups;
   long long* trace;
@@ -126,6 +135,7 @@
   if (p.diag) {
     TrapRecord* d = p.diag;
     d->tag = tag, d->stage = stage, d->bx = blockIdx.x, d->by = blockIdx.y, d->bz = blockIdx.z, d->rank = (int)cluster_ctarank();
+    d->peer = p.pair ? d->rank ^ 1 : -1;
     d->M = p.M, d->N = p.N, d->K = p.K, d->bn = p.bn, d->mode = p.mode, d->splits = p.splits, d->conv = p.conv;
     __threadfence_system();
     d->magic = TRAP_MAGIC;
@@ -171,77 +181,55 @@
   }
 }
 
-__device__ __forceinline__ void epilogue_chunk(const GemmParams& p, const uint32_t (&r)[32], int row, int64_t crow, int col0) {
-  const __half* rb = p.rowbias ? p.rowbias + (int64_t)(row / p.rows_per_group) * p.rowbias_ld : nullptr;
-  if (p.act == 3) {
-    if (col0 >= p.N) return;
-    float v[16];
-#pragma unroll
-    for (int e = 0; e < 16; ++e) {
-      float a = __uint_as_float(r[e]) * p.alpha, g = __uint_as_float(r[16 + e]) * p.alpha;
-      if (p.bias) a += __ldg(p.bias + col0 + e), g += __ldg(p.bias + col0 + 16 + e);
-      v[e] = a * gelu_erf(g);
-    }
-    const int64_t o = crow + (col0 >> 1);
-    float lo[8], hi[8];
-#pragma unroll
-    for (int e = 0; e < 8; ++e) lo[e] = v[e], hi[e] = v[8 + e];
-    store8(p, o, lo);
-    store8(p, o + 8, hi);
-    return;
-  }
-#pragma unroll
-  for (int j = 0; j < 32; j += 8) {
-    const int col = col0 + j;
-    if (col >= p.N) break;
-    float v[8];
-    const bool full = col + 8 <= p.N;
-    if (full && rb) {
-      uint4 q = *reinterpret_cast<const uint4*>(rb + col);
-      const __half* h = reinterpret_cast<const __half*>(&q);
-#pragma unroll
-      for (int e = 0; e < 8; ++e) v[e] = __half2float(h[e]);
-    } else {
-#pragma unroll
-      for (int e = 0; e < 8; ++e) v[e] = (rb && col + e < p.N) ? __half2float(rb[col + e]) : 0.f;
-    }
-#pragma unroll
-    for (int e = 0; e < 8; ++e) {
-      float x = fmaf(__uint_as_float(r[j + e]), p.alpha, v[e]);
-      if (p.bias && col + e < p.N) x += __ldg(p.bias + col + e);
-      v[e] = apply_act(x, p.act);
-    }
-    if (full && (p.ldc & 7) == 0) {
-      if (p.residual) {
-        uint4 q = *reinterpret_cast<const uint4*>(p.residual + crow + col);
-        const __half* h = reinterpret_cast<const __half*>(&q);
-#pragma unroll
-        for (int e = 0; e < 8; ++e) v[e] += __half2float(h[e]);
-      }
-      store8(p, crow + col, v);
-    } else {
-      for (int e = 0; e < 8 && col + e < p.N; ++e) {
-        float x = v[e];
-        if (p.residual) x += __half2float(p.residual[crow + col + e]);
-        if (p.out_f32) reinterpret_cast<float*>(p.C)[crow + col + e] = x;
-        else reinterpret_cast<__half*>(p.C)[crow + col + e] = __float2half_rn(x);
-      }
-    }
-  }
-}
-
-__device__ __forceinline__ void splitk_partial(const GemmParams& p, const uint32_t (&r)[32], int split, int row, int col0) {
-  float* w = p.ws + ((int64_t)split * p.M + row) * p.N + col0;
-  if ((p.N & 3) == 0) {
-#pragma unroll
-    for (int e = 0; e < 32; e += 4)
-      if (col0 + e < p.N)
-        __stcg(reinterpret_cast<float4*>(w + e), make_float4(__uint_as_float(r[e]), __uint_as_float(r[e + 1]),
-                                                              __uint_as_float(r[e + 2]), __uint_as_float(r[e + 3])));
-  } else {
-#pragma unroll
-    for (int e = 0; e < 32; ++e)
-      if (col0 + e < p.N) __stcg(w + e, __uint_as_float(r[e]));
+template <int BN>
+__device__ __forceinline__ void epilogue_generic(const GemmParams& p, const float (&d)[BN / 2], int wg, int t, int m0, int n0, int bz,
+                                                 bool split) {
+  const int cq = frag_col(t);
+#pragma unroll
+  for (int h = 0; h < 2; ++h) {
+    const int row = m0 + 64 * wg + frag_row(t) + 8 * h;
+    if (row >= p.M) continue;
+    if (split) {
+      float* w = p.ws + ((int64_t)bz * p.M + row) * p.N;
+#pragma unroll
+      for (int j = 0; j < BN / 8; ++j) {
+        const int col = n0 + 8 * j + cq;
+        if ((p.N & 1) == 0) {
+          if (col < p.N) __stcg(reinterpret_cast<float2*>(w + col), make_float2(d[4 * j + 2 * h], d[4 * j + 2 * h + 1]));
+        } else {
+          if (col < p.N) __stcg(w + col, d[4 * j + 2 * h]);
+          if (col + 1 < p.N) __stcg(w + col + 1, d[4 * j + 2 * h + 1]);
+        }
+      }
+      continue;
+    }
+    const int64_t crow = (p.batched ? (int64_t)(bz % p.nh) * p.stride_c_h + (int64_t)(bz / p.nh) * p.stride_c_b : 0) + out_row(p, row) * p.ldc;
+    const __half* rb = p.rowbias ? p.rowbias + (int64_t)(row / p.rows_per_group) * p.rowbias_ld : nullptr;
+#pragma unroll
+    for (int j = 0; j < BN / 8; ++j) {
+#pragma unroll
+      for (int e = 0; e < 2; ++e) {
+        const int col = n0 + 8 * j + cq + e;
+        if (col >= p.N) continue;
+        float x;
+        if (p.act == 3) {
+          if ((j & 3) >= 2) continue;
+          float a = d[4 * j + 2 * h + e] * p.alpha, g = d[4 * (j + 2) + 2 * h + e] * p.alpha;
+          if (p.bias) a += __ldg(p.bias + col), g += __ldg(p.bias + col + 16);
+          x = a * gelu_erf(g);
+          const int64_t o = crow + ((col - (col & 31)) >> 1) + (col & 15);
+          if (p.out_f32) reinterpret_cast<float*>(p.C)[o] = x;
+          else reinterpret_cast<__half*>(p.C)[o] = __float2half_rn(x);
+          continue;
+        }
+        x = fmaf(d[4 * j + 2 * h + e], p.alpha, rb ? __half2float(rb[col]) : 0.f);
+        if (p.bias) x += __ldg(p.bias + col);
+        x = apply_act(x, p.act);
+        if (p.residual) x += __half2float(p.residual[crow + col]);
+        if (p.out_f32) reinterpret_cast<float*>(p.C)[crow + col] = x;
+        else reinterpret_cast<__half*>(p.C)[crow + col] = __float2half_rn(x);
+      }
+    }
   }
 }
 
@@ -378,44 +366,53 @@
   return x;
 }
 
-template <int ACT>
-__device__ __forceinline__ void stage_rows(const GemmParams& p, const float* acc_row, uint8_t* mine, int n0, int c_lo, int c_hi,
-                                           const float* sbias, const __half* rb, bool rb_smem) {
-#pragma unroll 1
-  for (int c0 = c_lo; c0 < c_hi; c0 += 32) {
-    if (n0 + c0 >= p.N) break;
-    uint32_t r[32];
-    acc_ld32(acc_row + c0, r);
-    if (ACT == 3) {
-      __half2 h[8];
-#pragma unroll
-      for (int e = 0; e < 16; e += 2) {
-        float a0 = fmaf(__uint_as_float(r[e]), p.alpha, sbias[c0 + e]), a1 = fmaf(__uint_as_float(r[e + 1]), p.alpha, sbias[c0 + e + 1]);
-        float g0 = fmaf(__uint_as_float(r[16 + e]), p.alpha, sbias[c0 + 16 + e]);
-        float g1 = fmaf(__uint_as_float(r[17 + e]), p.alpha, sbias[c0 + 17 + e]);
-        h[e >> 1] = __floats2half2_rn(a0 * gelu_erf_fast(g0), a1 * gelu_erf_fast(g1));
-      }
-      uint4* d = reinterpret_cast<uint4*>(mine + (c0 - c_lo));
-      d[0] = reinterpret_cast<uint4*>(h)[0], d[1] = reinterpret_cast<uint4*>(h)[1];
+__host__ __device__ constexpr int epi_slab_row_bytes(int bn) { return col_split(bn) * 2 + 16; }
+
+template <int BN, int ACT>
+__device__ __forceinline__ void stage_frag(const GemmParams& p, const float (&d)[BN / 2], uint8_t* slabs, int wg, int t, int m0, int n0,
+                                           const float* sbias, const __half* srb) {
+  constexpr int CSPLIT = col_split(BN);
+  constexpr bool GEGLU = ACT == 3;
+  constexpr int STRIDE_LO = (GEGLU ? CSPLIT / 2 : CSPLIT) * 2 + 16, STRIDE_HI = (GEGLU ? (BN - CSPLIT) / 2 : BN - CSPLIT) * 2 + 16;
+  const int tr = 64 * wg + frag_row(t), cq = frag_col(t);
+  const int q = tr >> 5, sr = tr & 31;
+  const __half* rb[2] = {nullptr, nullptr};
+  bool rb_smem = false;
+  if (!GEGLU && p.rowbias) {
+    const int g0 = m0 / p.rows_per_group, last = (m0 + BM - 1 < p.M ? m0 + BM - 1 : p.M - 1) / p.rows_per_group;
+    rb_smem = last - g0 + 1 <= EPI_RB_GROUPS;
+#pragma unroll
+    for (int h = 0; h < 2; ++h) {
+      const int rr = m0 + tr + 8 * h < p.M ? m0 + tr + 8 * h : p.M - 1;
+      rb[h] = rb_smem ? srb + (rr / p.rows_per_group - g0) * BN : p.rowbias + (int64_t)(rr / p.rows_per_group) * p.rowbias_ld + n0;
+    }
+  }
+#pragma unroll
+  for (int j = 0; j < BN / 8; ++j) {
+    if (GEGLU && (j & 3) >= 2) continue;
+    const bool hi = 8 * j >= CSPLIT;
+    const int stride = hi ? STRIDE_HI : STRIDE_LO;
+    const int c = 8 * j + cq, lc = c - (hi ? CSPLIT : 0);
+    uint8_t* dst = slabs + (hi ? q + 4 : q) * (32 * epi_slab_row_bytes(BN)) + sr * stride;
+    if (GEGLU) {
+      const int oc = ((lc - (lc & 31)) >> 1) + (lc & 15);
+#pragma unroll
+      for (int h = 0; h < 2; ++h) {
+        const float a0 = fmaf(d[4 * j + 2 * h], p.alpha, sbias[c]), a1 = fmaf(d[4 * j + 2 * h + 1], p.alpha, sbias[c + 1]);
+        const float g0 = fmaf(d[4 * j + 8 + 2 * h], p.alpha, sbias[c + 16]), g1 = fmaf(d[4 * j + 9 + 2 * h], p.alpha, sbias[c + 17]);
+        *reinterpret_cast<__half2*>(dst + 8 * h * stride + oc * 2) = __floats2half2_rn(a0 * gelu_erf_fast(g0), a1 * gelu_erf_fast(g1));
+      }
     } else {
-#pragma unroll
-      for (int j = 0; j < 32; j += 8) {
-        float v[8];
-        const float4 b0 = *reinterpret_cast<const float4*>(sbias + c0 + j), b1 = *reinterpret_cast<const float4*>(sbias + c0 + j + 4);
-        v[0] = b0.x, v[1] = b0.y, v[2] = b0.z, v[3] = b0.w, v[4] = b1.x, v[5] = b1.y, v[6] = b1.z, v[7] = b1.w;
-        if (rb && (rb_smem || n0 + c0 + j + 8 <= p.N)) {
-          uint4 q = *reinterpret_cast<const uint4*>(rb + c0 + j);
-          const __half* hq = reinterpret_cast<const __half*>(&q);
-#pragma unroll
-          for (int e = 0; e < 8; ++e) v[e] += __half2float(hq[e]);
+      const float2 b = *reinterpret_cast<const float2*>(sbias + c);
+#pragma unroll
+      for (int h = 0; h < 2; ++h) {
+        float v0 = b.x, v1 = b.y;
+        if (rb[h] && (rb_smem || n0 + c < p.N)) {
+          const float2 r = __half22float2(*reinterpret_cast<const __half2*>(rb[h] + c));
+          v0 += r.x, v1 += r.y;
         }
-        __half2 h[4];
-#pragma unroll
-        for (int e = 0; e < 8; e += 2) {
-          float x0 = fmaf(__uint_as_float(r[j + e]), p.alpha, v[e]), x1 = fmaf(__uint_as_float(r[j + e + 1]), p.alpha, v[e + 1]);
-          h[e >> 1] = __floats2half2_rn(act_fn<ACT>(x0), act_fn<ACT>(x1));
-        }
-        *reinterpret_cast<uint4*>(mine + (c0 - c_lo + j) * 2) = *reinterpret_cast<uint4*>(h);
+        const float x0 = fmaf(d[4 * j + 2 * h], p.alpha, v0), x1 = fmaf(d[4 * j + 2 * h + 1], p.alpha, v1);
+        *reinterpret_cast<__half2*>(dst + 8 * h * stride + lc * 2) = __floats2half2_rn(act_fn<ACT>(x0), act_fn<ACT>(x1));
       }
     }
   }
@@ -463,31 +460,8 @@
 }
 
 template <int BN, int MODE>
-__device__ __forceinline__ void epilogue_staged(const GemmParams& p, const WarpOut& g, const float* acc_row, uint8_t* slab, int lane,
-                                                int m0, int row0, int n0, int c_lo, int c_hi, const float* sbias, const __half* srb,
-                                                const uint4 (&resq)[RES_PREFETCH]) {
-  const int row = row0 + lane;
-  const __half* rb = nullptr;
-  bool rb_smem = false;
-  if (MODE != 1 && p.rowbias) {
-    const int rr = row < p.M ? row : p.M - 1;
-    const int g0 = m0 / p.rows_per_group, last = (m0 + BM - 1 < p.M ? m0 + BM - 1 : p.M - 1) / p.rows_per_group;
-    rb_smem = last - g0 + 1 <= EPI_RB_GROUPS;
-    rb = rb_smem ? srb + (rr / p.rows_per_group - g0) * BN : p.rowbias + (int64_t)(rr / p.rows_per_group) * p.rowbias_ld + n0;
-  }
-  uint8_t* mine = slab + lane * g.stride;
-  if (MODE == 0) {
-    stage_rows<0>(p, acc_row, mine, n0, c_lo, c_hi, sbias, rb, rb_smem);
-  } else if (MODE == 1) {
-    stage_rows<3>(p, acc_row, mine, n0, c_lo, c_hi, sbias, rb, rb_smem);
-  } else {
-    switch (p.act) {
-      case 1: stage_rows<1>(p, acc_row, mine, n0, c_lo, c_hi, sbias, rb, rb_smem); break;
-      case 2: stage_rows<2>(p, acc_row, mine, n0, c_lo, c_hi, sbias, rb, rb_smem); break;
-      default: stage_rows<4>(p, acc_row, mine, n0, c_lo, c_hi, sbias, rb, rb_smem); break;
-    }
-  }
-  __syncwarp();
+__device__ __forceinline__ void epilogue_store(const GemmParams& p, const WarpOut& g, uint8_t* slab, int lane, int row0,
+                                               const uint4 (&resq)[RES_PREFETCH]) {
   __half* C = reinterpret_cast<__half*>(p.C);
 #pragma unroll
   for (int u = 0; u < RES_PREFETCH; ++u) {
@@ -564,37 +538,36 @@
   }
 }
 
-__host__ __device__ constexpr int epi_slab_bytes(int bn) { return EPI_WARPS * 32 * (col_split(bn) * 2 + 16); }
+__host__ __device__ constexpr int epi_slab_bytes(int bn) { return EPI_WARPS * 32 * epi_slab_row_bytes(bn); }
+constexpr int SMEM_LIMIT = 227 * 1024;
 constexpr int smem_bytes(int bn, int stages) {
   return stages * (BM * BK * 2 + bn * BK * 2) + epi_slab_bytes(bn) + 2 * stages * 8 + 16 + epi_smem_bytes(bn) + 1024;
 }
+constexpr int ring_stages(int bn) {
+  int s = 1;
+  while (smem_bytes(bn, s + 1) <= SMEM_LIMIT) ++s;
+  return s;
+}
 
 template <int BN>
 __device__ __forceinline__ void produce_stage(const GemmParams& p, const CUtensorMap* tmA, const CUtensorMap* tmB, uint8_t* a_dst,
-                                              uint8_t* b_dst, uint64_t* full_bar, int kb, int m0, int n0, int bz) {
+                                              uint8_t* b_dst, uint64_t* full_bar, int kb, int m0, int n0, int bz, int rank) {
   mbar_expect_tx(full_bar, BM * BK * 2 + BN * BK * 2);
+  int kc = kb * BK;
   if (p.conv) {
     const int tap = kb / p.cblocks, c0 = (kb - tap * p.cblocks) * BK;
     const int x0 = m0 % p.cW, y0 = (m0 / p.cW) % p.cH, b0 = m0 / (p.cW * p.cH);
     tma_load_4d(a_dst, tmA, full_bar, c0, x0 + tap % p.ctx + p.cox, y0 + tap / p.ctx + p.coy, b0);
-    tma_load_2d(b_dst, tmB, full_bar, tap * p.cC + c0, n0);
+    kc = tap * p.cC + c0;
   } else if (p.batched) {
     tma_load_4d(a_dst, tmA, full_bar, kb * BK, m0, bz % p.nh, bz / p.nh);
     tma_load_4d(b_dst, tmB, full_bar, kb * BK, n0, bz % p.nh, bz / p.nh);
+    return;
   } else {
     tma_load_2d(a_dst, tmA, full_bar, kb * BK, m0);
-    tma_load_2d(b_dst, tmB, full_bar, kb * BK, n0);
-  }
-}
-
-template <int BN>
-__device__ __forceinline__ void acc_store(float* acc, const float (&d)[BN / 2], int row0, int t) {
-  const int r = row0 + 16 * (t >> 5) + ((t & 31) >> 2), c = 2 * (t & 3);
-#pragma unroll
-  for (int j = 0; j < BN / 8; ++j) {
-    *reinterpret_cast<float2*>(acc + r * acc_ld(BN) + 8 * j + c) = make_float2(d[4 * j], d[4 * j + 1]);
-    *reinterpret_cast<float2*>(acc + (r + 8) * acc_ld(BN) + 8 * j + c) = make_float2(d[4 * j + 2], d[4 * j + 3]);
-  }
+  }
+  if (p.pair) tma_load_2d_mc(b_dst + rank * (BN / 2) * BK * 2, tmB, full_bar, kc, n0 + rank * (BN / 2), 0x3);
+  else tma_load_2d(b_dst, tmB, full_bar, kc, n0);
 }
 
 template <int BN, int STAGES, int MODE>
@@ -603,9 +576,8 @@
   extern __shared__ __align__(1024) uint8_t smem_raw[];
   uint8_t* smem = reinterpret_cast<uint8_t*>((reinterpret_cast<uintptr_t>(smem_raw) + 1023) & ~(uintptr_t)1023);
   constexpr int A_BYTES = BM * BK * 2, B_BYTES = BN * BK * 2;
-  static_assert(B_BYTES % 1024 == 0, "stage bases must stay 1024-byte aligned for SWIZZLE_128B");
-  static_assert(BN % 32 == 0 && BN >= 64 && BN <= 256, "tile width: a multiple of 32 (GEGLU chunks, 32-column epilogue reads)");
-  static_assert(BM * acc_ld(BN) * 4 <= STAGES * (A_BYTES + B_BYTES), "the accumulator tile must fit in the operand ring");
+  static_assert(B_BYTES % 2048 == 0, "stage bases and the pair's B halves must stay 1024-byte aligned for SWIZZLE_128B");
+  static_assert(BN % 32 == 0 && BN >= 64 && BN <= 256, "tile width: a multiple of 32 (GEGLU chunks: value and gate in one tile)");
   constexpr int CSPLIT = col_split(BN);
   uint8_t* sA = smem;
   uint8_t* sB = smem + STAGES * A_BYTES;
@@ -614,7 +586,6 @@
   uint64_t* empty = full + STAGES;
   float* sbias = reinterpret_cast<float*>((reinterpret_cast<uintptr_t>(empty + STAGES) + 15) & ~(uintptr_t)15);
   __half* srb = reinterpret_cast<__half*>(sbias + BN);
-  float* acc = reinterpret_cast<float*>(smem);
 
   const int warp = threadIdx.x >> 5, lane = threadIdx.x & 31;
   if (threadIdx.x == 0) stamp(p, 0), stamp_ns(p, 16);
@@ -626,102 +597,101 @@
     kb0 = (int)((int64_t)nk * bz / p.splits);
     kb1 = (int)((int64_t)nk * (bz + 1) / p.splits);
   }
+  const bool pair = MODE != 3 && p.pair;
+  const int csz = pair ? 2 : 1, rank = pair ? (int)cluster_ctarank() : 0;
 
   if (threadIdx.x == 0) {
     asm volatile("prefetch.tensormap [%0];" ::"l"(&tmA) : "memory");
     asm volatile("prefetch.tensormap [%0];" ::"l"(&tmB) : "memory");
-    for (int s = 0; s < STAGES; ++s) mbar_init(full + s, 1), mbar_init(empty + s, 2);
+    for (int s = 0; s < STAGES; ++s) mbar_init(full + s, 1), mbar_init(empty + s, 2 * csz);
     asm volatile("fence.mbarrier_init.release.cluster;" ::: "memory");
     asm volatile("fence.proxy.async.shared::cta;" ::: "memory");
   }
-  __syncthreads();
+  if (pair) cluster_sync_all();
+  else __syncthreads();
   pdl_wait();
   pdl_trigger();
   if (threadIdx.x == 0) stamp(p, 1);
 
-  const int tiles_m = (p.M + BM - 1) / BM, tiles = tiles_m * ((p.N + BN - 1) / BN);
+  const int tiles_m = (p.M + BM - 1) / BM, slots_m = (tiles_m + csz - 1) / csz, units = slots_m * ((p.N + BN - 1) / BN);
   const bool persist = MODE != 3 && p.persist;
   uint32_t cnt = 0;
-  for (int t = persist ? blockIdx.x : blockIdx.y * tiles_m + blockIdx.x; t < tiles; t += persist ? gridDim.x : tiles) {
-  const int m0 = (t % tiles_m) * BM, n0 = (t / tiles_m) * BN;
+  for (int u = persist ? blockIdx.x / csz : blockIdx.y * slots_m + blockIdx.x / csz; u < units; u += persist ? gridDim.x / csz : units) {
+  const int m0 = ((u % slots_m) * csz + rank) * BM, n0 = (u / slots_m) * BN;
   if (warp < 4) {
     if (threadIdx.x == 0) {
-      asm volatile("fence.proxy.async.shared::cta;" ::: "memory");
       for (int kb = kb0; kb < kb1; ++kb) {
         const uint32_t c = cnt + (kb - kb0);
         const int s = c % STAGES;
         const uint32_t ph = (c / STAGES) & 1;
         mbar_wait(empty + s, ph ^ 1, p, WAIT_EMPTY, s);
-        produce_stage<BN>(p, &tmA, &tmB, sA + s * A_BYTES, sB + s * B_BYTES, full + s, kb, m0, n0, bz);
+        produce_stage<BN>(p, &tmA, &tmB, sA + s * A_BYTES, sB + s * B_BYTES, full + s, kb, m0, n0, bz, rank);
         if (kb == kb0) stamp(p, 2);
       }
       stamp(p, 3);
     }
     __syncwarp();
   } else {
-    const int wg = (warp >> 2) - 1, e = warp - 4, quarter = e & 3, te = threadIdx.x - 128;
+    const int wg = (warp >> 2) - 1, e = warp - 4, quarter = e & 3, te = threadIdx.x - 128, t = threadIdx.x & 127;
     const int c_lo = e < 4 ? 0 : CSPLIT, c_hi = e < 4 ? CSPLIT : BN;
     const int row0 = m0 + quarter * 32;
-    if (MODE != 3) epilogue_preload<BN>(p, m0, n0, sbias, srb, te);
-    {
-      float d[BN / 2];
-#pragma unroll
-      for (int i = 0; i < BN / 2; ++i) d[i] = 0.f;
-      for (int kb = kb0; kb < kb1; ++kb) {
-        const uint32_t c = cnt + (kb - kb0);
-        const int s = c % STAGES;
-        const uint32_t ph = (c / STAGES) & 1;
-        mbar_wait(full + s, ph, p, WAIT_FULL, s);
-        if (kb == kb0 && te == 0) stamp(p, 4);
-        const uint32_t a0 = smem_u32(sA + s * A_BYTES) + wg * (64 * 128), b0 = smem_u32(sB + s * B_BYTES);
-        wg::fence();
-#pragma unroll
-        for (int k = 0; k < BK / 16; ++k)
-          wg::mma_f16<BN>(d, wg::desc_sw128(a0 + k * 32), wg::desc_sw128(b0 + k * 32), 1);
-        wg::commit();
-        wg::wait<1>();
-        if (kb > kb0 && (threadIdx.x & 127) == 0) mbar_arrive(empty + (c - 1) % STAGES);
-      }
-      wg::wait<0>();
-      if ((threadIdx.x & 127) == 0) mbar_arrive(empty + (cnt + kb1 - kb0 - 1) % STAGES);
-      if (te == 0) stamp(p, 5);
-      epi_bar();
-      acc_store<BN>(acc, d, 64 * wg, threadIdx.x & 127);
-    }
-    epi_bar();
-    if (te == 0) stamp(p, 6);
-    const float* acc_row = acc + (quarter * 32 + lane) * acc_ld(BN);
+    const bool live = m0 < p.M;
+    if (MODE != 3 && live) epilogue_preload<BN>(p, m0, n0, sbias, srb, te);
+    auto release = [&](int s) {
+      if (t == 0) {
+        mbar_arrive(empty + s);
+        if (pair) mbar_arrive_remote(empty + s, rank ^ 1);
+      }
+    };
+    float d[BN / 2];
+#pragma unroll
+    for (int i = 0; i < BN / 2; ++i) d[i] = 0.f;
+    for (int kb = kb0; kb < kb1; ++kb) {
+      const uint32_t c = cnt + (kb - kb0);
+      const int s = c % STAGES;
+      const uint32_t ph = (c / STAGES) & 1;
+      mbar_wait(full + s, ph, p, WAIT_FULL, s);
+      if (kb == kb0 && te == 0) stamp(p, 4);
+      const uint32_t a0 = smem_u32(sA + s * A_BYTES) + wg * (64 * 128), b0 = smem_u32(sB + s * B_BYTES);
+      wg::fence();
+#pragma unroll
+      for (int k = 0; k < BK / 16; ++k)
+        wg::mma_f16<BN>(d, wg::desc_sw128(a0 + k * 32), wg::desc_sw128(b0 + k * 32), 1);
+      wg::commit();
+      wg::wait<1>();
+      if (kb > kb0) release((c - 1) % STAGES);
+    }
+    wg::wait<0>();
+    release((cnt + kb1 - kb0 - 1) % STAGES);
+    if (te == 0) stamp(p, 5);
     if (MODE != 3) {
-      const WarpOut g = warp_out<MODE>(p, n0, c_lo, c_hi);
-      uint4 resq[RES_PREFETCH];
-      prefetch_residual(p, g, lane, row0, resq);
-      epilogue_staged<BN, MODE>(p, g, acc_row, slabs + e * 32 * (CSPLIT * 2 + 16), lane, m0, row0, n0, c_lo, c_hi, sbias, srb, resq);
+      if (live) {
+        if (MODE == 0) {
+          stage_frag<BN, 0>(p, d, slabs, wg, t, m0, n0, sbias, srb);
+        } else if (MODE == 1) {
+          stage_frag<BN, 3>(p, d, slabs, wg, t, m0, n0, sbias, srb);
+        } else {
+          switch (p.act) {
+            case 1: stage_frag<BN, 1>(p, d, slabs, wg, t, m0, n0, sbias, srb); break;
+            case 2: stage_frag<BN, 2>(p, d, slabs, wg, t, m0, n0, sbias, srb); break;
+            default: stage_frag<BN, 4>(p, d, slabs, wg, t, m0, n0, sbias, srb); break;
+          }
+        }
+        const WarpOut g = warp_out<MODE>(p, n0, c_lo, c_hi);
+        uint4 resq[RES_PREFETCH];
+        prefetch_residual(p, g, lane, row0, resq);
+        epi_bar();
+        if (te == 0) stamp(p, 6);
+        epilogue_store<BN, MODE>(p, g, slabs + e * 32 * epi_slab_row_bytes(BN), lane, row0, resq);
+      }
     } else {
-      const int row = row0 + lane;
-      if (split) {
-        if (te == 0) stamp_ns(p, 17);
-#pragma unroll 1
-        for (int c0 = c_lo; c0 < c_hi; c0 += 32) {
-          uint32_t r[32];
-          acc_ld32(acc_row + c0, r);
-          if (row < p.M) splitk_partial(p, r, bz, row, n0 + c0);
-        }
-        if (te == 0) stamp_ns(p, 18);
-      } else {
-        const int64_t crow = (p.batched ? (int64_t)(bz % p.nh) * p.stride_c_h + (int64_t)(bz / p.nh) * p.stride_c_b : 0) +
-                             out_row(p, row < p.M ? row : 0) * p.ldc;
-#pragma unroll 1
-        for (int c0 = c_lo; c0 < c_hi; c0 += 32) {
-          uint32_t r[32];
-          acc_ld32(acc_row + c0, r);
-          if (row < p.M) epilogue_chunk(p, r, row, crow, n0 + c0);
-        }
-      }
+      if (split && te == 0) stamp_ns(p, 17);
+      epilogue_generic<BN>(p, d, wg, t, m0, n0, bz, split);
+      if (split && te == 0) stamp_ns(p, 18);
     }
     if (te == 0) stamp(p, 7);
   }
   cnt += kb1 - kb0;
-  __syncthreads();
   }
   if (split) {
     cluster_sync_all();
@@ -731,6 +701,7 @@
       if (threadIdx.x == 128) stamp_ns(p, 22, true);
     }
   }
+  if (pair) cluster_sync_all();
   if (threadIdx.x == 0) stamp(p, 8);
 }
 
@@ -789,11 +760,13 @@
 struct Config {
   int bn, splits;
   int persist;
+  int pair;
 };
 
 int g_force[3] = {-1, 0, 0};
 int g_persist = 0;
 int g_persist_min_tiles = 0;
+int g_pair = 0;
 void read_force_env() {
   if (g_force[0] >= 0) return;
   g_force[0] = g_force[1] = g_force[2] = 0;
@@ -823,11 +796,19 @@
   return us;
 }
 
+int pick_mode(const GemmParams& p, const Config& c) {
+  const int nout = p.act == 3 ? p.N / 2 : p.N;
+  const bool staged = !p.out_f32 && c.splits <= 1 && !p.batched && (nout % 8) == 0 && (p.ldc % 8) == 0 && ((uintptr_t)p.C % 16) == 0 &&
+                      (!p.residual || ((uintptr_t)p.residual % 16) == 0);
+  if (!staged) return 3;
+  return p.act == 0 ? 0 : (p.act == 3 ? 1 : 2);
+}
+
 Config pick_config(const GemmParams& p, int nk, bool can_split, int64_t ws_floats) {
   read_force_env();
   Config c;
   const int M = p.M, N = p.N;
-  c.persist = 0;
+  c.persist = 0, c.pair = 0;
   if (p.batched) {
     c.bn = N <= 64 ? 64 : 128, c.splits = 1;
     return c;
@@ -854,26 +835,19 @@
     c.bn = (g_force[1] == 64 || g_force[1] == 128 || g_force[1] == 160 || g_force[1] == 256) ? g_force[1] : 128;
     c.splits = 1;
   }
+  c.pair = g_pair == 1 && c.splits == 1 && pick_mode(p, c) != 3;
   const int tiles = cdiv(M, BM) * cdiv(N, c.bn);
   const int min_tiles = g_persist_min_tiles > 0 ? g_persist_min_tiles : 4 * sm_count();
   c.persist = c.splits == 1 && (g_persist == 1 || (g_persist == 0 && tiles >= min_tiles));
   return c;
 }
 
-int pick_mode(const GemmParams& p, const Config& c) {
-  const int nout = p.act == 3 ? p.N / 2 : p.N;
-  const bool staged = !p.out_f32 && c.splits <= 1 && !p.batched && (nout % 8) == 0 && (p.ldc % 8) == 0 && ((uintptr_t)p.C % 16) == 0 &&
-                      (!p.residual || ((uintptr_t)p.residual % 16) == 0);
-  if (!staged) return 3;
-  return p.act == 0 ? 0 : (p.act == 3 ? 1 : 2);
-}
-
 long long* g_trace = nullptr;
 
 template <int BN, int STAGES, int MODE>
-int launch(const CUtensorMap& a, const CUtensorMap& b, GemmParams p, int batch, int persist, cudaStream_t st) {
+int launch(const CUtensorMap& a, const CUtensorMap& b, GemmParams p, int batch, int persist, int pair, cudaStream_t st) {
   constexpr int SMEM = smem_bytes(BN, STAGES);
-  static_assert(SMEM <= 227 * 1024, "one CTA per SM");
+  static_assert(SMEM <= SMEM_LIMIT, "one CTA per SM");
   static PerDeviceOnce attr;
   if (attr.need())
     O2345_CUDA(cudaFuncSetAttribute(gemm_tc_kernel<BN, STAGES, MODE>, cudaFuncAttributeMaxDynamicSharedMemorySize, SMEM));
@@ -881,24 +855,49 @@
   p.diag = diag_buffer(st);
   const int splits = (MODE == 3 && batch == 0 && p.splits > 1) ? p.splits : 1;
   p.splits = splits;
-  dim3 grid(cdiv(p.M, BM), cdiv(p.N, BN), batch > 0 ? batch : splits);
+  p.pair = MODE != 3 && batch == 0 && splits == 1 && pair;
+  const int csz = p.pair ? 2 : 1;
+  dim3 grid(csz * cdiv(cdiv(p.M, BM), csz), cdiv(p.N, BN), batch > 0 ? batch : splits);
   p.persist = MODE != 3 && batch == 0 && splits == 1 && persist;
   if (p.persist) {
-    const int tiles = (int)grid.x * (int)grid.y;
-    grid = dim3(tiles < sm_count() ? tiles : sm_count(), 1, 1);
-  }
-  O2345_CUDA(launch_pdl_cluster(gemm_tc_kernel<BN, STAGES, MODE>, grid, dim3(GEMM_THREADS), (size_t)SMEM, st, 1, splits, a, b, p));
+    int cap = sm_count();
+    if (p.pair) {
+      static int clusters[64] = {0};
+      int dev = 0;
+      O2345_CUDA(cudaGetDevice(&dev));
+      if (dev < 0 || dev >= 64 || clusters[dev] == 0) {
+        cudaLaunchConfig_t cfg;
+        memset(&cfg, 0, sizeof(cfg));
+        cfg.gridDim = dim3(2 * sm_count()), cfg.blockDim = dim3(GEMM_THREADS), cfg.dynamicSmemBytes = SMEM;
+        cudaLaunchAttribute at;
+        at.id = cudaLaunchAttributeClusterDimension;
+        at.val.clusterDim.x = 2, at.val.clusterDim.y = 1, at.val.clusterDim.z = 1;
+        cfg.attrs = &at, cfg.numAttrs = 1;
+        int n = 0;
+        O2345_CUDA(cudaOccupancyMaxActiveClusters(&n, gemm_tc_kernel<BN, STAGES, MODE>, &cfg));
+        if (n < 1) { set_error("gemm_tc_kernel<BN=%d>: no CTA pair fits on an SM pair", BN); return O2345_ECUDA; }
+        if (dev >= 0 && dev < 64) clusters[dev] = n;
+        cap = n;
+      } else {
+        cap = clusters[dev];
+      }
+    }
+    const int units = (int)grid.x / csz * (int)grid.y;
+    grid = dim3(csz * (units < cap ? units : cap), 1, 1);
+  }
+  O2345_CUDA(launch_pdl_cluster(gemm_tc_kernel<BN, STAGES, MODE>, grid, dim3(GEMM_THREADS), (size_t)SMEM, st, csz, splits, a, b, p));
   O2345_LAUNCH_CHECK();
   return O2345_OK;
 }
 
 template <int BN, int STAGES>
-int launch_mode(int mode, const CUtensorMap& a, const CUtensorMap& b, const GemmParams& p, int batch, int persist, cudaStream_t st) {
+int launch_mode(int mode, const CUtensorMap& a, const CUtensorMap& b, const GemmParams& p, int batch, int persist, int pair,
+                cudaStream_t st) {
   switch (mode) {
-    case 0: return launch<BN, STAGES, 0>(a, b, p, batch, persist, st);
-    case 1: return launch<BN, STAGES, 1>(a, b, p, batch, persist, st);
-    case 2: return launch<BN, STAGES, 2>(a, b, p, batch, persist, st);
-    default: return launch<BN, STAGES, 3>(a, b, p, batch, persist, st);
+    case 0: return launch<BN, STAGES, 0>(a, b, p, batch, persist, pair, st);
+    case 1: return launch<BN, STAGES, 1>(a, b, p, batch, persist, pair, st);
+    case 2: return launch<BN, STAGES, 2>(a, b, p, batch, persist, pair, st);
+    default: return launch<BN, STAGES, 3>(a, b, p, batch, persist, pair, st);
   }
 }
 
@@ -907,17 +906,17 @@
     set_error("o2345_gemm_f16: column statistics need the staged fp16 epilogue (16-byte aligned C / residual) or split-K");
     return O2345_EUNSUPPORTED;
   }
-  if (c.bn == 64) return launch_mode<64, 6>(mode, a, b, p, batch, c.persist, st);
-  if (c.bn == 128) return launch_mode<128, 5>(mode, a, b, p, batch, c.persist, st);
-  if (c.bn == 160) return launch_mode<160, 4>(mode, a, b, p, batch, c.persist, st);
-  return launch_mode<256, 3>(mode, a, b, p, batch, c.persist, st);
+  if (c.bn == 64) return launch_mode<64, ring_stages(64)>(mode, a, b, p, batch, c.persist, c.pair, st);
+  if (c.bn == 128) return launch_mode<128, ring_stages(128)>(mode, a, b, p, batch, c.persist, c.pair, st);
+  if (c.bn == 160) return launch_mode<160, ring_stages(160)>(mode, a, b, p, batch, c.persist, c.pair, st);
+  return launch_mode<256, ring_stages(256)>(mode, a, b, p, batch, c.persist, c.pair, st);
 }
 
 int fill_epilogue(GemmParams& p, const o2345_epilogue* ep, int M, int N, int64_t ldc) {
   p.bias = nullptr, p.rowbias = nullptr, p.rowbias_ld = 0, p.rows_per_group = 1, p.residual = nullptr;
   p.out_f32 = 0, p.act = 0, p.alpha = 1.f, p.trace = g_trace;
   p.colstats = nullptr, p.stats_rpg = 1, p.stats_groups = 0;
-  p.diag = nullptr, p.bn = p.mode = 0;
+  p.diag = nullptr, p.bn = p.mode = 0, p.persist = p.pair = 0;
   if (!ep) return O2345_OK;
   O2345_CHECK_ARG(ep->act >= 0 && ep->act <= 4, "unknown activation");
   O2345_CHECK_ARG(!ep->rowbias || (ep->rows_per_group > 0 && (ep->rowbias_ld % 8) == 0 && ((uintptr_t)ep->rowbias % 16) == 0),
@@ -954,6 +953,8 @@
 
 extern "C" void o2345_debug_gemm_persist(int mode, int min_tiles) { g_persist = mode, g_persist_min_tiles = min_tiles; }
 
+extern "C" void o2345_debug_gemm_pair(int mode) { g_pair = mode; }
+
 extern "C" void o2345_debug_gemm_model(const float* seven) {
   for (int i = 0; i < 7; ++i) g_model[i] = seven[i];
 }
@@ -966,9 +967,9 @@
   static const char* names[] = {"?", "empty (producer waiting for the MMA to free a stage)", "full (MMA issuer waiting for TMA bytes)",
                                 };
   snprintf(buf, n,
-           "gemm_tc_kernel<BN=%d, MODE=%d> M=%d N=%d K=%d conv=%d splits=%d: CTA (%d,%d,%d) rank %d gave up after 4 s "
+           "gemm_tc_kernel<BN=%d, MODE=%d> M=%d N=%d K=%d conv=%d splits=%d: CTA (%d,%d,%d) rank %d (peer %d) gave up after 4 s "
            "on barrier '%s' stage %d",
-           d->bn, d->mode, d->M, d->N, d->K, d->conv, d->splits, d->bx, d->by, d->bz, d->rank,
+           d->bn, d->mode, d->M, d->N, d->K, d->conv, d->splits, d->bx, d->by, d->bz, d->rank, d->peer,
            names[d->tag >= 1 && d->tag <= 2 ? d->tag : 0], d->stage);
   return 1;
 }
@@ -1002,7 +1003,7 @@
   set_workspace(p, splitk_ws, ws_floats);
   const Config c = pick_config(p, taps * p.cblocks, true, ws_floats);
   p.splits = c.splits;
-  rc = make_map(&mb, weight, N, taps * (int64_t)C, taps * (int64_t)C, 0, 0, 0, 0, c.bn);
+  rc = make_map(&mb, weight, N, taps * (int64_t)C, taps * (int64_t)C, 0, 0, 0, 0, c.pair ? c.bn / 2 : c.bn);
   if (rc) return rc;
   return dispatch(c, pick_mode(p, c), ma, mb, p, 0, st);
 }
@@ -1068,7 +1069,7 @@
   CUtensorMap ma, mb;
   rc = make_map(&ma, A, M, K, lda, nh, nb, stride_a_h, stride_a_b, BM);
   if (rc) return rc;
-  rc = make_map(&mb, B, N, K, ldb, nh, nb, stride_b_h, stride_b_b, c.bn);
+  rc = make_map(&mb, B, N, K, ldb, nh, nb, stride_b_h, stride_b_b, c.pair ? c.bn / 2 : c.bn);
   if (rc) return rc;
   return dispatch(c, pick_mode(p, c), ma, mb, p, nh > 0 ? nh * nb : 0, st);
 }
diff --git a/one-2-3-45_b200/o2345/_lib.py b/one-2-3-45_b200/o2345/_lib.py
--- a/one-2-3-45_b200/o2345/_lib.py
+++ b/one-2-3-45_b200/o2345/_lib.py
@@ -87,6 +87,7 @@
     "o2345_debug_gemm_trace": (None, [c_fp]),
     "o2345_debug_gemm_force": (None, [C.c_int, C.c_int, C.c_int]),
     "o2345_debug_gemm_persist": (None, [C.c_int, C.c_int]),
+    "o2345_debug_gemm_pair": (None, [C.c_int]),
     "o2345_debug_groupnorm_cluster": (None, [C.c_int]),
     "o2345_debug_gemm_model": (None, [C.POINTER(C.c_float)]),
     "o2345_last_trap": (C.c_int, [C.c_char_p, C.c_size_t]),
```
